# h22hyeon/PC-GNN

Measured on AMD Instinct MI355X. Metric: sampled-nodes/sec, higher is better.
Workload: dtype f32; 1 GPU; yelpchi-like N=45954 F=32 R=3 edges=49315/573616/3402743 endpoints=pareto(2.0) x uniform, PCGNN emb=64 batch=1024 rho=0.5, pick 2*|train_pos|=5346/epoch; global_batch=1024, parallelism=single, engine=graph, epochs_per_launch=4, nodes_processed=1741546

## Files before the change

### pc-gnn_amd/csrc/select.hip

```cpp
#include <limits.h>
#include <stdlib.h>

#include "choose.h"
#include "dense.h"

namespace pcg {

constexpr int KEY_UNROLL = 8;
template <int LEVEL>
__device__ __forceinline__ float s0_ld(const float *__restrict__ s0, uint32_t id) {
    return s0[id];
}
constexpr int KPT = T1_CAP / PCG_WAVE;

#define PCG_STAMP(slot)                                                                \
    do {                                                                               \
        if (a.stamps && tid == 0) a.stamps[(size_t)row * 8 + (slot)] = wall_clock64(); \
    } while (0)

template <int NW>
__device__ __forceinline__ void grp_sync() {
    if constexpr (NW > 1) __syncthreads();
}

template <int NW>
__device__ __forceinline__ void grp_scan(int v, int wave, int lane, int *red, int &prefix, int &total) {
    if constexpr (NW == 1) {
        prefix = 0;
        total = v;
    } else {
        if (lane == 0) red[wave] = v;
        __syncthreads();
        int p = 0, t = 0;
#pragma unroll
        for (int w = 0; w < NW; ++w) {
            const int x = red[w];
            if (w < wave) p += x;
            t += x;
        }
        __syncthreads();
        prefix = p;
        total = t;
    }
}

__device__ __forceinline__ uint32_t wave_min_u32(uint32_t v) {
    uint32_t t;
    t = dpp_u32<0xB1>(v); v = t < v ? t : v;
    t = dpp_u32<0x4E>(v); v = t < v ? t : v;
    t = dpp_u32<0x141>(v); v = t < v ? t : v;
    t = dpp_u32<0x140>(v); v = t < v ? t : v;
    const uint32_t r0 = (uint32_t)__builtin_amdgcn_readlane((int)v, 0), r1 = (uint32_t)__builtin_amdgcn_readlane((int)v, 16);
    const uint32_t r2 = (uint32_t)__builtin_amdgcn_readlane((int)v, 32), r3 = (uint32_t)__builtin_amdgcn_readlane((int)v, 48);
    const uint32_t x = r0 < r1 ? r0 : r1, y = r2 < r3 ? r2 : r3;
    return x < y ? x : y;
}
__device__ __forceinline__ uint32_t wave_max_u32(uint32_t v) {
    uint32_t t;
    t = dpp_u32<0xB1>(v); v = t > v ? t : v;
    t = dpp_u32<0x4E>(v); v = t > v ? t : v;
    t = dpp_u32<0x141>(v); v = t > v ? t : v;
    t = dpp_u32<0x140>(v); v = t > v ? t : v;
    const uint32_t r0 = (uint32_t)__builtin_amdgcn_readlane((int)v, 0), r1 = (uint32_t)__builtin_amdgcn_readlane((int)v, 16);
    const uint32_t r2 = (uint32_t)__builtin_amdgcn_readlane((int)v, 32), r3 = (uint32_t)__builtin_amdgcn_readlane((int)v, 48);
    const uint32_t x = r0 > r1 ? r0 : r1, y = r2 > r3 ? r2 : r3;
    return x > y ? x : y;
}
__device__ __forceinline__ bool sorted_contains(const uint32_t *list, int n, uint32_t x) {
    int lo = 0, hi = n;
    while (lo < hi) {
        const int mid = (lo + hi) >> 1;
        if (list[mid] < x) lo = mid + 1;
        else hi = mid;
    }
    return lo < n && list[lo] == x;
}

constexpr int SORT_SPIN_MAX = 1 << 21;
constexpr int KIDX_MAX = 512;
__device__ __forceinline__ uint64_t pk_ld(const uint64_t *pk, int i);
__device__ __forceinline__ void wait_sorted_keys(const ChooseArgs &a, int &keys_ok, int lane, int *sortw) {
    if (a.n_sort == 0 || keys_ok) return;
    if (__hip_atomic_load(&sortw[0], __ATOMIC_ACQUIRE, __HIP_MEMORY_SCOPE_WORKGROUP) == 0) {
        int elected = 0;
        if (lane == 0) elected = atomicCAS(&sortw[1], 0, 1) == 0;
        elected = __builtin_amdgcn_readfirstlane(elected);
        if (elected) {
            for (int spins = 0;; ++spins) {
                const unsigned seen = (unsigned)__builtin_amdgcn_readfirstlane(
                    (int)__hip_atomic_load(a.sort_done, __ATOMIC_RELAXED, __HIP_MEMORY_SCOPE_AGENT));
                if (seen >= (unsigned)a.n_sort) break;
                if (spins >= SORT_SPIN_MAX) {
                    if (lane == 0 && a.status) atomicOr(a.status, (uint32_t)PCG_ST_SYNC_TIMEOUT);
                    break;
                }
                __builtin_amdgcn_s_sleep(4);
            }
            __builtin_amdgcn_fence(__ATOMIC_ACQUIRE, "workgroup");
            const int P = a.g.n_pos;
            int stride = 16;
            while ((P + stride - 1) / stride > KIDX_MAX) stride <<= 1;
            const int n_idx = (P + stride - 1) / stride;
            for (int t = lane; t < n_idx; t += PCG_WAVE) sortw[4 + t] = (int)(uint32_t)(pk_ld(a.pos_keys, t * stride) >> 32);
            if (lane == 0) {
                sortw[2] = n_idx;
                sortw[3] = stride;
            }
            if (lane == 0) __hip_atomic_store(&sortw[0], 1, __ATOMIC_RELEASE, __HIP_MEMORY_SCOPE_WORKGROUP);
        } else {
            while (__hip_atomic_load(&sortw[0], __ATOMIC_ACQUIRE, __HIP_MEMORY_SCOPE_WORKGROUP) == 0) __builtin_amdgcn_s_sleep(2);
        }
    }
    __builtin_amdgcn_fence(__ATOMIC_ACQUIRE, "workgroup");
    keys_ok = 1;
}

#ifndef PCG_PK_NT
#define PCG_PK_NT 2
#endif
__device__ __forceinline__ uint64_t pk_ld(const uint64_t *pk, int i) {
#if PCG_PK_NT == 2
    const __amdgpu_buffer_rsrc_t rsrc = __builtin_amdgcn_make_buffer_rsrc(const_cast<uint64_t *>(pk), 0, 0x7FFFFFFF, 0x00020000);
    typedef unsigned int u2 __attribute__((ext_vector_type(2)));
    const u2 v = __builtin_amdgcn_raw_buffer_load_b64(rsrc, i * 8, 0, 16);
    return ((uint64_t)v.y << 32) | v.x;
#elif PCG_PK_NT == 1
    return __builtin_nontemporal_load(pk + i);
#else
    return pk[i];
#endif
}

__device__ __forceinline__ float pos_score(const uint64_t *pk, int i) { return from_orderable((uint32_t)(pk_ld(pk, i) >> 32)); }
__device__ __forceinline__ uint32_t pos_dkey(const uint64_t *pk, int i, float c) { return dist_key(c, pos_score(pk, i)); }

template <class Pred>
__device__ __forceinline__ int wave_partition_point(int lo, int hi, int lane, Pred pred) {
    for (;;) {
        const int n = hi - lo;
        if (n <= 0) return lo;
        if (n <= PCG_WAVE) {
            const int idx = lo + lane;
            return lo + wave_count(idx < hi && pred(idx));
        }
        const int step = (n + PCG_WAVE - 1) >> 6;
        int q = lo + (lane + 1) * step - 1;
        if (q > hi - 1) q = hi - 1;
        const int c = wave_count(pred(q));
        if (c == PCG_WAVE) return hi;
        int qc = lo + (c + 1) * step - 1;
        if (qc > hi - 1) qc = hi - 1;
        if (c > 0) {
            int ql = lo + c * step - 1;
            if (ql > hi - 1) ql = hi - 1;
            lo = ql + 1;
        }
        hi = qc;
    }
}

__device__ __forceinline__ int run_end_fwd(const uint64_t *pk, float c, uint32_t kstar, int i0, int end, int lane) {
    for (int i = i0; i < end; i += PCG_WAVE) {
        const int j = i + lane;
        const bool same = j < end && pos_dkey(pk, j, c) == kstar;
        const uint64_t bad = ~__ballot(same);
        if (bad) {
            const int f = i + (__ffsll((unsigned long long)bad) - 1);
            return f < end ? f : end;
        }
    }
    return end;
}
__device__ __forceinline__ int run_begin_bwd(const uint64_t *pk, float c, uint32_t kstar, int i0, int low, int lane) {
    for (int i = i0; i >= low; i -= PCG_WAVE) {
        const int j = i - lane;
        const bool same = j >= low && pos_dkey(pk, j, c) == kstar;
        const uint64_t bad = ~__ballot(same);
        if (bad) {
            const int f = i - (__ffsll((unsigned long long)bad) - 1);
            return (f >= low ? f : low - 1) + 1;
        }
    }
    return low;
}

__device__ __forceinline__ void wave_kth(uint32_t ck, bool have, int n, int want, uint32_t &kstar, int &need, int &n_equal) {
    int lt = 0, eq = 0;
    for (int j = 0; j < n; ++j) {
        const uint32_t o = (uint32_t)__builtin_amdgcn_readlane((int)ck, j);
        lt += o < ck;
        eq += o == ck;
    }
    const int r = want - 1;
    const uint64_t hit = __ballot(have && lt <= r && r < lt + eq);
    const int src = hit ? __ffsll((unsigned long long)hit) - 1 : 0;
    kstar = (uint32_t)__builtin_amdgcn_readlane((int)ck, src);
    n_equal = __builtin_amdgcn_readlane(eq, src);
    need = want - __builtin_amdgcn_readlane(lt, src);
}

struct MinorWindow {
    int L, R, L2, R2, tau, need_t;
};
__device__ __forceinline__ MinorWindow minority_window(const ChooseArgs &a, int m, float c, int lane, const int *sortw) {
    const uint64_t *__restrict__ pk = a.pos_keys;
    const int P = a.g.n_pos;
    int L, R, L2, R2, tau = INT_MAX, need_t = 0;
    if (m >= P) {
        L = L2 = 0;
        R = R2 = P;
    } else {
        int lo_min = 0, lo_max = P - m;
        if (a.n_sort > 0 && sortw) {
            const int n_idx = sortw[2], stride = sortw[3];
            const uint32_t *ix = reinterpret_cast<const uint32_t *>(sortw + 4);
            const int t = wave_partition_point(0, n_idx, lane, [&](int x) { return from_orderable(ix[x]) < c; });
            const int pc_lo = t > 0 ? (t - 1) * stride + 1 : 0, pc_hi = t * stride < P ? t * stride : P;
            lo_min = pc_lo - m > 0 ? pc_lo - m : 0;
            lo_max = pc_hi < P - m ? pc_hi : P - m;
            lo_max = lo_max < lo_min ? lo_min : lo_max;
        }
        const int lo = wave_partition_point(lo_min, lo_max, lane, [&](int x) {
            return (c - pos_score(pk, x)) > (pos_score(pk, x + m) - c);
        });
        const uint32_t NOKEY = 0xFFFFFFFEu;
        const uint32_t ka = pos_dkey(pk, lo, c), kb = pos_dkey(pk, lo + m - 1, c);
        const uint32_t ka1 = m > 1 ? pos_dkey(pk, lo + 1, c) : NOKEY;
        const uint32_t kb1 = m > 1 ? pos_dkey(pk, lo + m - 2, c) : NOKEY;
        const uint32_t kl = lo > 0 ? pos_dkey(pk, lo - 1, c) : NOKEY;
        const uint32_t kr = lo + m < P ? pos_dkey(pk, lo + m, c) : NOKEY;
        const uint32_t ks = ka > kb ? ka : kb;
        const bool tie_l = ka == ks, tie_r = kb == ks;
        const bool none_outside = kl != ks && kr != ks;
        if (none_outside && m == 1) {
            L2 = lo;
            L = R = R2 = lo + 1;
        } else if (none_outside && !(tie_l && tie_r) && (tie_l ? ka1 != ks : kb1 != ks)) {
            L2 = L = tie_l ? lo + 1 : lo;
            R = R2 = tie_l ? lo + m : lo + m - 1;
            if (tie_l) L2 = lo; else R2 = lo + m;
        } else {
            L = run_end_fwd(pk, c, ks, lo, lo + m, lane);
            R = (L == lo + m) ? L : run_begin_bwd(pk, c, ks, lo + m - 1, L, lane);
            L2 = run_begin_bwd(pk, c, ks, lo - 1, 0, lane);
            R2 = run_end_fwd(pk, c, ks, lo + m, P, lane);
        }
        need_t = m - (R - L);
        const int T = (L - L2) + (R2 - R);
        if (T == need_t) {
            L = L2;
            R = R2;
            need_t = 0;
        } else if (T > PCG_WAVE) {
            int plo = 0, phi = P - 1;
            while (plo < phi) {
                const int mid = (plo + phi) >> 1;
                int cn = 0;
                for (int i0 = L2; i0 < L; i0 += PCG_WAVE) {
                    const int i = i0 + lane;
                    cn += wave_count(i < L && (int)(uint32_t)pk_ld(pk, i) <= mid);
                }
                for (int i0 = R; i0 < R2; i0 += PCG_WAVE) {
                    const int i = i0 + lane;
                    cn += wave_count(i < R2 && (int)(uint32_t)pk_ld(pk, i) <= mid);
                }
                if (cn >= need_t) phi = mid;
                else plo = mid + 1;
            }
            tau = plo;
        } else {
            const int nl = L - L2;
            const int ti = lane < nl ? L2 + lane : R + (lane - nl);
            const bool tv = lane < T;
            const int tp = tv ? (int)(uint32_t)pk_ld(pk, ti) : INT_MAX;
            int rank = 0;
            for (int j = 0; j < T; ++j) rank += __builtin_amdgcn_readlane(tp, j) < tp;
            const uint64_t hit = __ballot(tv && rank == need_t - 1);
            const int src = __ffsll((unsigned long long)hit) - 1;
            tau = __builtin_amdgcn_readlane(tp, src < 0 ? 0 : src);
        }
    }
    MinorWindow w;
    w.L = L; w.R = R; w.L2 = L2; w.R2 = R2; w.tau = tau; w.need_t = need_t;
    return w;
}

template <int NW>
__device__ __forceinline__ void finish_row(const ChooseArgs &a, int row, const RowRec &p, float c, const uint32_t *sel, int ns,
                                           bool sel_stored, int wave, int lane, int *red, int &keys_ok, int *sortw,
                                           const int *pre_window = nullptr) {
    constexpr int NT = NW * PCG_WAVE;
    const int tid = wave * PCG_WAVE + lane;
    const int m = p.m, node = p.node;
    int32_t *__restrict__ out = a.w.list + p.lbeg;
    int mt = 0;
    int valid = 0;
    if (m > 0) {
        const uint64_t *__restrict__ pk = a.pos_keys;
        int L, R, L2, R2, tau, need_t;
        if (pre_window) {
            L = pre_window[0]; R = pre_window[1]; L2 = pre_window[2]; R2 = pre_window[3]; tau = pre_window[4]; need_t = pre_window[5];
        } else {
            wait_sorted_keys(a, keys_ok, lane, sortw);
            PCG_STAMP(7);
            const MinorWindow mw = minority_window(a, m, c, lane, sortw);
            L = mw.L; R = mw.R; L2 = mw.L2; R2 = mw.R2; tau = mw.tau; need_t = mw.need_t;
        }
        PCG_STAMP(4);
        const int n_strict = R - L;
        for (int base = tid; base < n_strict; base += NT * KEY_UNROLL) {
            uint32_t pos[KEY_UNROLL], u[KEY_UNROLL];
#pragma unroll
            for (int x = 0; x < KEY_UNROLL; ++x) {
                const int j = base + x * NT;
                pos[x] = (uint32_t)pk_ld(pk, L + (j < n_strict ? j : n_strict - 1));
            }
#pragma unroll
            for (int x = 0; x < KEY_UNROLL; ++x) u[x] = (uint32_t)a.g.train_pos[pos[x]];
#pragma unroll
            for (int x = 0; x < KEY_UNROLL; ++x) {
                const int j = base + x * NT;
                if (j < n_strict) {
                    const bool dup = sorted_contains(sel, ns, u[x]) || (a.add_self && u[x] == (uint32_t)node);
                    out[ns + j] = dup ? -1 : (int32_t)u[x];
                    valid += !dup;
                }
            }
        }
        mt = n_strict;
        if (need_t > 0) {
            int taken = 0;
            for (int part = 0; part < 2; ++part) {
                const int s0i = part == 0 ? L2 : R, e0i = part == 0 ? L : R2;
                for (int i0 = s0i; i0 < e0i; i0 += PCG_WAVE) {
                    const int i = i0 + lane;
                    bool take = false;
                    uint32_t u = 0;
                    if (i < e0i) {
                        const uint32_t pos = (uint32_t)pk_ld(pk, i);
                        take = (int)pos <= tau;
                        if (take) u = (uint32_t)a.g.train_pos[pos];
                    }
                    const uint64_t tmk = __ballot(take);
                    if (take && wave == 0) {
                        const bool dup = sorted_contains(sel, ns, u) || (a.add_self && u == (uint32_t)node);
                        out[ns + n_strict + taken + __popcll(tmk & lanemask_lt())] = dup ? -1 : (int32_t)u;
                        valid += !dup;
                    }
                    taken += __popcll(tmk);
                }
            }
            mt += taken;
        }
    }
    PCG_STAMP(5);
    int n_self = 0;
    if (a.add_self && !sorted_contains(sel, ns, (uint32_t)node)) {
        n_self = 1;
        if (tid == 0) out[ns + mt] = node;
    }
    int vsum = valid;
    for (int o = 1; o < PCG_WAVE; o <<= 1) vsum += __shfl_xor(vsum, o);
    int vpre, vtot;
    grp_scan<NW>(vsum, wave, lane, red, vpre, vtot);
    if (!sel_stored)
        for (int i = tid; i < ns; i += NT) out[i] = (int32_t)sel[i];
    const int used = ns + mt + n_self;
    const int nch = (rec_cap(p, a.add_self) + CHUNK - 1) / CHUNK;
    for (int j = tid; j < nch; j += NT) {
        const int left = used - j * CHUNK;
        a.w.chunk_desc[p.chunk0 + j].z = left < 0 ? 0 : (left > CHUNK ? CHUNK : left);
    }
    if (tid == 0) {
        a.w.len[row] = used;
        a.cnt[row] = ns + vtot + n_self;
    }
    grp_sync<NW>();
    PCG_STAMP(6);
}

__device__ __forceinline__ void report_plain_row(const ChooseArgs &a, int row, const RowRec &p, int ns) {
    a.w.len[row] = ns;
    a.cnt[row] = ns;
    const int nch = (rec_cap(p, 0) + CHUNK - 1) / CHUNK;
    for (int j = 0; j < nch; ++j) {
        const int left = ns - j * CHUNK;
        a.w.chunk_desc[p.chunk0 + j].z = left < 0 ? 0 : (left > CHUNK ? CHUNK : left);
    }
}

#define PCG_ROR_STEP(N)                                                                                     \
    do {                                                                                                    \
        const uint32_t ok = (uint32_t)__builtin_amdgcn_update_dpp(0, (int)key, 0x120 + (N), 0xF, 0xF, false); \
        const int op = __builtin_amdgcn_update_dpp(0, pos, 0x120 + (N), 0xF, 0xF, false);                  \
        rank += (ok < key) || (ok == key && op < pos);                                                      \
    } while (0)

__device__ __forceinline__ void select_four_short_rows(const ChooseArgs &a, int q_first, int na, const int32_t *const *t_indices,
                                                       int lane) {
    const int g = lane >> 4, pos = lane & 15;
    const int qi = q_first + g;
    const bool active = qi < na;
    const int row = a.w.qa[active ? qi : na - 1];
    const RowRec p = a.w.recs[row];
    const int r = row / a.B;
    const int32_t *__restrict__ nbr = t_indices[r] + (p.d > 0 ? p.start : 0);
    const bool have = active && pos < p.d;
    const uint32_t id = (uint32_t)nbr[pos < p.d ? pos : (p.d > 0 ? p.d - 1 : 0)];
    const float c = a.center_s0 ? a.center_s0[row - r * a.B] : a.s0[p.node + a.center_off];
    const bool keep_all = rec_keep_all(p);
    const float sc = s0_ld<2>(a.s0, id);
    const uint32_t key = have ? dist_key(c, sc) : 0xFFFFFFFFu;
    int rank = 0;
    PCG_ROR_STEP(1); PCG_ROR_STEP(2); PCG_ROR_STEP(3); PCG_ROR_STEP(4); PCG_ROR_STEP(5);
    PCG_ROR_STEP(6); PCG_ROR_STEP(7); PCG_ROR_STEP(8); PCG_ROR_STEP(9); PCG_ROR_STEP(10);
    PCG_ROR_STEP(11); PCG_ROR_STEP(12); PCG_ROR_STEP(13); PCG_ROR_STEP(14); PCG_ROR_STEP(15);
    const bool sel = have && (keep_all || rank < p.k);
    const uint32_t gm = (uint32_t)(__ballot(sel) >> (16 * g)) & 0xFFFFu;
    if (sel) a.w.list[p.lbeg + __popc(gm & ((1u << pos) - 1u))] = (int32_t)id;
    if (active && pos == 0) report_plain_row(a, row, p, __popc(gm));
}

__device__ __forceinline__ void select_lane_row(const ChooseArgs &a, int row, uint32_t *area, int lane, int &keys_ok, int *sortw) {
    const int tid = lane;
    if (a.stamps && tid == 0) a.stamps[(size_t)row * 8] = wall_clock64() | ((unsigned long long)blockIdx.x << 54);
    const RowRec p = a.w.recs[row];
    const int d = p.d, k = p.k;
    const bool keep_all = rec_keep_all(p);
    const int r = row / a.B;
    const int32_t *__restrict__ nbr = a.g.indices[r] + (d > 0 ? p.start : 0);
    const float c = a.center_s0 ? a.center_s0[row - r * a.B] : a.s0[p.node + a.center_off];
    uint32_t *sel_lds = area + HIST_W;
    const bool tail = p.m > 0 || a.add_self;
    const bool have = lane < d;
    const uint32_t id = (uint32_t)nbr[have ? lane : (d > 0 ? d - 1 : 0)];
    const float sc = s0_ld<2>(a.s0, id);
    const uint32_t mine = have ? dist_key(c, sc) : 0xFFFFFFFFu;
    PCG_STAMP(1);
    int rank = 0;
    if (!keep_all) {
        for (int j = 0; j < d; ++j)
            rank += (uint32_t)__builtin_amdgcn_readlane((int)mine, j) < mine;
        int sum = have ? rank : 0;
        sum += (int)dpp_u32<0xB1>((uint32_t)sum);
        sum += (int)dpp_u32<0x4E>((uint32_t)sum);
        sum += (int)dpp_u32<0x141>((uint32_t)sum);
        sum += (int)dpp_u32<0x140>((uint32_t)sum);
        const int total = __builtin_amdgcn_readlane(sum, 0) + __builtin_amdgcn_readlane(sum, 16) +
                          __builtin_amdgcn_readlane(sum, 32) + __builtin_amdgcn_readlane(sum, 48);
        if (total != d * (d - 1) / 2)
            for (int j = 0; j < d; ++j)
                rank += ((uint32_t)__builtin_amdgcn_readlane((int)mine, j) == mine) && j < lane;
    }
    const bool s = have && (keep_all || rank < k);
    const uint64_t sm = __ballot(s);
    const int ns = __popcll(sm);
    PCG_STAMP(2);
    if (s) {
        const int at = __popcll(sm & lanemask_lt());
        if (tail) sel_lds[at] = id;
        else a.w.list[p.lbeg + at] = (int32_t)id;
    }
    PCG_STAMP(3);
    if (tail) finish_row<1>(a, row, p, c, sel_lds, ns, false, 0, lane, nullptr, keys_ok, sortw);
    else {
        if (lane == 0) report_plain_row(a, row, p, ns);
        PCG_STAMP(6);
    }
}

__device__ __forceinline__ void select_wave_row(const ChooseArgs &a, int row, uint32_t *area, int lane, int &keys_ok, int *sortw) {
    const int tid = lane;
    if (a.stamps && tid == 0) a.stamps[(size_t)row * 8] = wall_clock64() | ((unsigned long long)blockIdx.x << 54);
    const RowRec p = a.w.recs[row];
    const int d = p.d, k = p.k;
    const bool keep_all = rec_keep_all(p);
    const int r = row / a.B;
    const int32_t *__restrict__ nbr = a.g.indices[r] + p.start;
    const float c = a.center_s0 ? a.center_s0[row - r * a.B] : a.s0[p.node + a.center_off];
    uint32_t *hist = area, *sel_lds = area + HIST_W, *cand = area + HIST_W + T1_CAP;
    const bool tail = p.m > 0 || a.add_self;
    int32_t *__restrict__ out = a.w.list + p.lbeg;

    uint32_t id[KPT], key[KPT];
    {
        float sc[KPT];
#pragma unroll
        for (int u = 0; u < KPT; ++u) {
            const int i = u * PCG_WAVE + lane;
            id[u] = (uint32_t)nbr[i < d ? i : d - 1];
        }
#pragma unroll
        for (int u = 0; u < KPT; ++u) sc[u] = s0_ld<2>(a.s0, id[u]);
#pragma unroll
        for (int u = 0; u < KPT; ++u) key[u] = (u * PCG_WAVE + lane < d) ? dist_key(c, sc[u]) : 0xFFFFFFFFu;
    }
    PCG_STAMP(1);

    uint32_t kstar = 0xFFFFFFFEu;
    int need = 0, n_equal = 0;
    if (!keep_all) {
        uint32_t kmin = 0xFFFFFFFFu, kmax = 0u;
#pragma unroll
        for (int u = 0; u < KPT; ++u)
            if (u * PCG_WAVE + lane < d) {
                kmin = key[u] < kmin ? key[u] : kmin;
                kmax = key[u] > kmax ? key[u] : kmax;
            }
        uint32_t lo = wave_min_u32(kmin), hi = wave_max_u32(kmax);
        int below = 0, cnt = d;
        while (lo < hi && cnt > PCG_WAVE) {
            const uint32_t range = hi - lo;
            const int bits = 32 - __clz((int)range);
            const int shift = bits > 8 ? bits - 8 : 0;
            *reinterpret_cast<uint4 *>(hist + 4 * lane) = make_uint4(0u, 0u, 0u, 0u);
#pragma unroll
            for (int u = 0; u < KPT; ++u)
                if (key[u] >= lo && key[u] <= hi) atomicAdd(&hist[(key[u] - lo) >> shift], 1u);
            const uint4 v = *reinterpret_cast<const uint4 *>(hist + 4 * lane);
            const int s = (int)(v.x + v.y + v.z + v.w);
            const int incl = wave_incl_scan(s, lane);
            const int want = k - below;
            const uint64_t reach = __ballot(incl >= want);
            const int L = __ffsll((unsigned long long)reach) - 1;
            int c0 = incl - s, b = 0, hb = (int)v.x;
            if (c0 + (int)v.x < want) {
                c0 += (int)v.x; b = 1; hb = (int)v.y;
                if (c0 + (int)v.y < want) {
                    c0 += (int)v.y; b = 2; hb = (int)v.z;
                    if (c0 + (int)v.z < want) { c0 += (int)v.z; b = 3; hb = (int)v.w; }
                }
            }
            const int bin = __builtin_amdgcn_readlane(4 * lane + b, L);
            below += __builtin_amdgcn_readlane(c0, L);
            cnt = __builtin_amdgcn_readlane(hb, L);
            lo += (uint32_t)bin << shift;
            const uint32_t top = lo + ((1u << shift) - 1u);
            hi = top < hi ? top : hi;
        }
        kstar = lo;
        need = k - below;
        n_equal = cnt;
        if (lo < hi) {
            int at = 0;
#pragma unroll
            for (int u = 0; u < KPT; ++u) {
                const bool isc = key[u] >= lo && key[u] <= hi;
                const uint64_t bm = __ballot(isc);
                if (isc) cand[at + __popcll(bm & lanemask_lt())] = key[u];
                at += __popcll(bm);
            }
            const bool hv = lane < cnt;
            const uint32_t ck = hv ? cand[lane] : 0xFFFFFFFFu;
            wave_kth(ck, hv, cnt, k - below, kstar, need, n_equal);
        }
    }
    PCG_STAMP(2);

    const bool ranked = n_equal != need;
    int ns = 0, ties_seen = 0;
#pragma unroll
    for (int u = 0; u < KPT; ++u) {
        if (u * PCG_WAVE >= d) break;
        const bool in = u * PCG_WAVE + lane < d;
        bool s = in && key[u] <= kstar;
        if (ranked) {
            const bool tie = in && key[u] == kstar;
            const uint64_t tm = __ballot(tie);
            s = in && (key[u] < kstar || (tie && ties_seen + __popcll(tm & lanemask_lt()) < need));
            ties_seen += __popcll(tm);
        }
        const uint64_t sm = __ballot(s);
        if (s) {
            const int at = ns + __popcll(sm & lanemask_lt());
            if (tail) sel_lds[at] = id[u];
            else out[at] = (int32_t)id[u];
        }
        ns += __popcll(sm);
    }
    PCG_STAMP(3);
    if (tail) finish_row<1>(a, row, p, c, sel_lds, ns, false, 0, lane, nullptr, keys_ok, sortw);
    else {
        if (lane == 0) report_plain_row(a, row, p, ns);
        PCG_STAMP(6);
    }
}

template <bool LDSK, class F>
__device__ __forceinline__ void for_keys(const uint32_t *keys, const uint32_t *__restrict__ gk, int first, int end, int step, F f) {
    if constexpr (LDSK) {
        for (int i = first; i < end; i += step) f(i, keys[i]);
    } else {
        for (int base = first; base < end; base += step * KEY_UNROLL) {
            uint32_t kv[KEY_UNROLL];
#pragma unroll
            for (int u = 0; u < KEY_UNROLL; ++u) {
                const int i = base + u * step;
                kv[u] = gk[i < end ? i : end - 1];
            }
#pragma unroll
            for (int u = 0; u < KEY_UNROLL; ++u) {
                const int i = base + u * step;
                if (i < end) f(i, kv[u]);
            }
        }
    }
}

template <bool LDSK, int NW = SEL_NW>
__device__ __forceinline__ void select_wg_row(const ChooseArgs &a, int row, uint32_t *keys, uint32_t *hist, uint32_t *cand,
                                              int *red, int tid, int &keys_ok, int *sortw, uint32_t *gk = nullptr,
                                              int key_cap = WG_KEYCAP ) {
    constexpr int NT = NW * PCG_WAVE;
    constexpr int HBITS = NW == 8 ? 11 : 12;
    static_assert(4 * NT == (1 << HBITS), "NW is 8 or 16");
    const int lane = tid & (PCG_WAVE - 1), wave = __builtin_amdgcn_readfirstlane(tid >> 6);
    if (a.stamps && tid == 0) a.stamps[(size_t)row * 8] = wall_clock64() | ((unsigned long long)blockIdx.x << 54);
    const RowRec p = a.w.recs[row];
    const int d = p.d, k = p.k;
    const bool keep_all = rec_keep_all(p);
    const int r = row / a.B;
    const int32_t *__restrict__ nbr = a.g.indices[r] + p.start;
    const float *__restrict__ s0 = a.s0;
    const float c = a.center_s0 ? a.center_s0[row - r * a.B] : s0[p.node + a.center_off];
    int32_t *__restrict__ out = a.w.list + p.lbeg;
    int *res = red + 2 * NW + 2;

    uint32_t kstar = 0xFFFFFFFFu;
    int need = 0, n_equal = 0;
    int *win = sortw ? sortw + 4 : nullptr;
    const bool early = !keep_all && p.m > 0 && a.n_sort == 0 && win != nullptr && NW > 1;
    if (!keep_all) {
        uint32_t kmin = 0xFFFFFFFFu, kmax = 0u;
        constexpr int KU1 = 16;
        const int nt1 = early ? NT - PCG_WAVE : NT;
        if (early && wave == NW - 1) {
            const MinorWindow mw = minority_window(a, p.m, c, lane, nullptr);
            if (lane == 0) {
                win[0] = mw.L; win[1] = mw.R; win[2] = mw.L2; win[3] = mw.R2; win[4] = mw.tau; win[5] = mw.need_t;
            }
        } else
        for (int base = tid; base < d; base += nt1 * KU1) {
            uint32_t id[KU1];
            float sc[KU1];
#pragma unroll
            for (int u = 0; u < KU1; ++u) {
                const int i = base + u * nt1;
                id[u] = (uint32_t)nbr[i < d ? i : d - 1];
            }
#pragma unroll
            for (int u = 0; u < KU1; ++u) sc[u] = s0_ld<1>(s0, id[u]);
#pragma unroll
            for (int u = 0; u < KU1; ++u) {
                const int i = base + u * nt1;
                if (i < d) {
                    const uint32_t key = dist_key(c, sc[u]);
                    if constexpr (LDSK) keys[i] = key;
                    else if (gk) gk[i] = key;
                    kmin = key < kmin ? key : kmin;
                    kmax = key > kmax ? key : kmax;
                }
            }
        }
        kmin = wave_min_u32(kmin);
        kmax = wave_max_u32(kmax);
        if (lane == 0) {
            red[wave] = (int)kmin;
            red[NW + wave] = (int)kmax;
        }
        if constexpr (!LDSK) __builtin_amdgcn_fence(__ATOMIC_RELEASE, "workgroup");
        __syncthreads();
        if constexpr (!LDSK) __builtin_amdgcn_fence(__ATOMIC_ACQUIRE, "workgroup");
        for (int w = 0; w < NW; ++w) {
            const uint32_t x = (uint32_t)red[w], y = (uint32_t)red[NW + w];
            kmin = x < kmin ? x : kmin;
            kmax = y > kmax ? y : kmax;
        }
        PCG_STAMP(1);
        uint32_t lo = kmin, hi = kmax;
        int below = 0, cnt = d;
        while (lo < hi && cnt > PCG_WAVE) {
            const uint32_t range = hi - lo;
            const int bits = 32 - __clz((int)range);
            const int shift = bits > HBITS ? bits - HBITS : 0;
            *reinterpret_cast<uint4 *>(hist + 4 * tid) = make_uint4(0u, 0u, 0u, 0u);
            __syncthreads();
            for_keys<LDSK>(keys, gk, tid, d, NT, [&](int, uint32_t key) {
                if (key >= lo && key <= hi) atomicAdd(&hist[(key - lo) >> shift], 1u);
            });
            __syncthreads();
            const uint4 v = *reinterpret_cast<const uint4 *>(hist + 4 * tid);
            const int s = (int)(v.x + v.y + v.z + v.w);
            const int incl_w = wave_incl_scan(s, lane);
            if (lane == PCG_WAVE - 1) red[wave] = incl_w;
            __syncthreads();
            int pre = 0;
#pragma unroll
            for (int w = 0; w < NW; ++w) pre += (w < wave) ? red[w] : 0;
            const int incl = pre + incl_w, excl = incl - s;
            const int want = k - below;
            if (excl < want && want <= incl) {
                int c0 = excl, b = 0, hb = (int)v.x;
                if (c0 + (int)v.x < want) {
                    c0 += (int)v.x; b = 1; hb = (int)v.y;
                    if (c0 + (int)v.y < want) {
                        c0 += (int)v.y; b = 2; hb = (int)v.z;
                        if (c0 + (int)v.z < want) { c0 += (int)v.z; b = 3; hb = (int)v.w; }
                    }
                }
                res[0] = 4 * tid + b;
                res[1] = c0;
                res[2] = hb;
            }
            __syncthreads();
            below += res[1];
            cnt = res[2];
            lo += (uint32_t)res[0] << shift;
            const uint32_t top = lo + ((1u << shift) - 1u);
            hi = top < hi ? top : hi;
        }
        kstar = lo;
        need = k - below;
        n_equal = cnt;
        if (lo < hi) {
            __syncthreads();
            if (tid == 0) res[3] = 0;
            __syncthreads();
            for_keys<LDSK>(keys, gk, tid, d, NT, [&](int, uint32_t key) {
                if (key >= lo && key <= hi) {
                    const int at = atomicAdd(&res[3], 1);
                    if (at < PCG_WAVE) cand[at] = key;
                }
            });
            __syncthreads();
            const bool hv = lane < cnt;
            const uint32_t ck = hv ? cand[lane] : 0xFFFFFFFFu;
            wave_kth(ck, hv, cnt, k - below, kstar, need, n_equal);
        }
        __syncthreads();
    }
    PCG_STAMP(2);

    const bool ranked = !keep_all && n_equal != need;
    const int seg = (((d + NW - 1) / NW) + PCG_WAVE - 1) & ~(PCG_WAVE - 1);
    const int b0 = wave * seg < d ? wave * seg : d;
    const int e0 = b0 + seg < d ? b0 + seg : d;
    int tie_base = 0;
    if (ranked) {
        int tc = 0;
        for_keys<LDSK>(keys, gk, b0 + lane, e0, PCG_WAVE, [&](int, uint32_t key) { tc += key == kstar; });
        for (int o = 1; o < PCG_WAVE; o <<= 1) tc += __shfl_xor(tc, o);
        int ttot;
        grp_scan<NW>(tc, wave, lane, red, tie_base, ttot);
    }
    int ns = 0;
    const bool plain = p.m == 0 && !a.add_self;
    const bool sel_in_lds = (LDSK || (keep_all ? d : k) <= key_cap) && !plain;
    uint32_t *selbuf = sel_in_lds ? keys : reinterpret_cast<uint32_t *>(out);
    if constexpr (LDSK) {
        uint32_t mask = 0;
        int mine = 0, ties_seen = tie_base;
        int it = 0;
        for (int i0 = b0; i0 < e0; i0 += PCG_WAVE, ++it) {
            const int i = i0 + lane;
            const bool in = i < e0;
            const uint32_t key = (in && !keep_all) ? keys[i] : 0u;
            bool s = in && (keep_all || key <= kstar);
            if (ranked) {
                const bool tie = in && key == kstar;
                const uint64_t tm = __ballot(tie);
                s = in && (key < kstar || (tie && ties_seen + __popcll(tm & lanemask_lt()) < need));
                ties_seen += __popcll(tm);
            }
            mask |= (uint32_t)s << it;
            mine += wave_count(s);
        }
        int run;
        grp_scan<NW>(mine, wave, lane, red, run, ns);
        constexpr int CU = 4;
        it = 0;
        for (int i0 = b0; i0 < e0; i0 += CU * PCG_WAVE, it += CU) {
            uint32_t idv[CU];
#pragma unroll
            for (int u = 0; u < CU; ++u) {
                const int i = i0 + u * PCG_WAVE + lane;
                idv[u] = (uint32_t)nbr[i < e0 ? i : d - 1];
            }
#pragma unroll
            for (int u = 0; u < CU; ++u) {
                const bool s = (mask >> (it + u)) & 1u;
                const uint64_t sm = __ballot(s);
                const int at = run + __popcll(sm & lanemask_lt());
                if (s) {
                    if (plain) out[at] = (int32_t)idv[u];
                    else keys[at] = idv[u];
                }
                run += __popcll(sm);
            }
        }
        __syncthreads();
    } else {
        auto stretch_keys = [&](int i0, uint32_t (&id)[KEY_UNROLL], uint32_t (&key)[KEY_UNROLL]) __attribute__((always_inline)) {
#pragma unroll
            for (int u = 0; u < KEY_UNROLL; ++u) {
                const int i = i0 + u * PCG_WAVE + lane;
                id[u] = (uint32_t)nbr[i < e0 ? i : d - 1];
                key[u] = gk[i < e0 ? i : d - 1];
            }
        };
        int mine = 0, ties_seen = tie_base;
        for (int i0 = b0; i0 < e0; i0 += PCG_WAVE * KEY_UNROLL) {
            uint32_t id[KEY_UNROLL], key[KEY_UNROLL];
            stretch_keys(i0, id, key);
#pragma unroll
            for (int u = 0; u < KEY_UNROLL; ++u) {
                const int i = i0 + u * PCG_WAVE + lane;
                const bool in = i < e0;
                bool s = in && (keep_all || key[u] <= kstar);
                if (ranked) {
                    const bool tie = in && key[u] == kstar;
                    const uint64_t tm = __ballot(tie);
                    s = in && (key[u] < kstar || (tie && ties_seen + __popcll(tm & lanemask_lt()) < need));
                    ties_seen += __popcll(tm);
                }
                mine += wave_count(s);
            }
        }
        int run;
        grp_scan<NW>(mine, wave, lane, red, run, ns);
        ties_seen = tie_base;
        for (int i0 = b0; i0 < e0; i0 += PCG_WAVE * KEY_UNROLL) {
            uint32_t id[KEY_UNROLL], key[KEY_UNROLL];
            stretch_keys(i0, id, key);
#pragma unroll
            for (int u = 0; u < KEY_UNROLL; ++u) {
                const int i = i0 + u * PCG_WAVE + lane;
                const bool in = i < e0;
                bool s = in && (keep_all || key[u] <= kstar);
                if (ranked) {
                    const bool tie = in && key[u] == kstar;
                    const uint64_t tm = __ballot(tie);
                    s = in && (key[u] < kstar || (tie && ties_seen + __popcll(tm & lanemask_lt()) < need));
                    ties_seen += __popcll(tm);
                }
                const uint64_t sm = __ballot(s);
                if (s) selbuf[run + __popcll(sm & lanemask_lt())] = id[u];
                run += __popcll(sm);
            }
        }
        __builtin_amdgcn_fence(__ATOMIC_RELEASE, "workgroup");
        __syncthreads();
        __builtin_amdgcn_fence(__ATOMIC_ACQUIRE, "workgroup");
    }
    PCG_STAMP(3);
    if (plain) {
        if (wave == 0) {
            if (lane == 0) {
                a.w.len[row] = ns;
                a.cnt[row] = ns;
            }
            const int nch = (rec_cap(p, 0) + CHUNK - 1) / CHUNK;
            for (int j = lane; j < nch; j += PCG_WAVE) {
                const int left = ns - j * CHUNK;
                a.w.chunk_desc[p.chunk0 + j].z = left < 0 ? 0 : (left > CHUNK ? CHUNK : left);
            }
        }
        PCG_STAMP(6);
        return;
    }
    if constexpr (LDSK) finish_row<NW>(a, row, p, c, keys, ns, false, wave, lane, red, keys_ok, sortw, early ? win : nullptr);
    else finish_row<NW>(a, row, p, c, selbuf, ns, !sel_in_lds, wave, lane, red, keys_ok, sortw, early ? win : nullptr);
}

#ifndef PCG_WG_ROW_PRIO
#define PCG_WG_ROW_PRIO 2
#endif
constexpr int SEL_SHARDS = 8;
constexpr int SORT_TILE = 4096;

template <int TILE, int NW = SEL_NW>
__device__ __forceinline__ void sort_share(const ChooseArgs &a, int w, uint64_t *sh, int *part, int tid) {
    static_assert(TILE % (NW * PCG_WAVE) == 0, "every thread loads the same number of keys of a tile");
    constexpr int PER = TILE / (NW * PCG_WAVE);
    const int lane = tid & (PCG_WAVE - 1), wave = tid >> 6;
    const int P = a.g.n_pos;
    const int group = w % a.n_sort, slice = w / a.n_sort;
    const int i = group * PCG_WAVE + lane;
    const uint64_t *__restrict__ raw = a.raw_keys;
    const uint64_t mine = raw[i < P ? i : P - 1] | (i < P ? 0ull : ~0ull);
    const int jb = slice * a.sort_slice_len;
    const int je = jb + a.sort_slice_len < P ? jb + a.sort_slice_len : P;
    int c = 0;
    for (int t0 = jb; t0 < je; t0 += TILE) {
        const int nt = je - t0 < TILE ? je - t0 : TILE;
        uint64_t kt[PER];
#pragma unroll
        for (int u = 0; u < PER; ++u) {
            const int t = tid + u * NW * PCG_WAVE;
            kt[u] = raw[t0 + (t < nt ? t : nt - 1)] | (t < nt ? 0ull : ~0ull);
        }
        __syncthreads();
#pragma unroll
        for (int u = 0; u < PER; ++u) sh[tid + u * NW * PCG_WAVE] = kt[u];
        __syncthreads();
        const int chunk = (((nt + NW - 1) / NW) + 7) & ~7;
        const int j0 = wave * chunk;
        const int nt8 = (nt + 7) & ~7;
        const int j1 = j0 + chunk < nt8 ? j0 + chunk : nt8;
        const uint4 *sh4 = reinterpret_cast<const uint4 *>(sh);
        for (int j = j0; j < j1; j += 8) {
            const uint4 q0 = sh4[(j >> 1) + 0], q1 = sh4[(j >> 1) + 1], q2 = sh4[(j >> 1) + 2], q3 = sh4[(j >> 1) + 3];
            const uint64_t a0 = ((uint64_t)q0.y << 32) | q0.x, a1 = ((uint64_t)q0.w << 32) | q0.z;
            const uint64_t a2 = ((uint64_t)q1.y << 32) | q1.x, a3 = ((uint64_t)q1.w << 32) | q1.z;
            const uint64_t a4 = ((uint64_t)q2.y << 32) | q2.x, a5 = ((uint64_t)q2.w << 32) | q2.z;
            const uint64_t a6 = ((uint64_t)q3.y << 32) | q3.x, a7 = ((uint64_t)q3.w << 32) | q3.z;
            c += (a0 < mine) + (a1 < mine) + (a2 < mine) + (a3 < mine) + (a4 < mine) + (a5 < mine) + (a6 < mine) + (a7 < mine);
        }
    }
    part[wave * PCG_WAVE + lane] = c;
    __syncthreads();
    if (wave == 0) {
        int cnt = 0;
#pragma unroll
        for (int x = 0; x < NW; ++x) cnt += part[x * PCG_WAVE + lane];
        uint32_t ticket = 0;
        if (a.sort_slices > 1) {
            if (i < P) __hip_atomic_fetch_add(a.rank_acc + i, (uint32_t)cnt, __ATOMIC_RELAXED, __HIP_MEMORY_SCOPE_AGENT);
            asm volatile("s_waitcnt vmcnt(0)" ::: "memory");
            if (lane == 0) ticket = __hip_atomic_fetch_add(a.group_ticket + group, 1u, __ATOMIC_RELAXED, __HIP_MEMORY_SCOPE_AGENT);
            ticket = (uint32_t)__builtin_amdgcn_readfirstlane((int)ticket);
        }
        if (ticket == (uint32_t)a.sort_slices - 1u) {
            if (i < P) {
                uint32_t rank = (uint32_t)cnt;
                if (a.sort_slices > 1) {
                    rank = __hip_atomic_load(a.rank_acc + i, __ATOMIC_RELAXED, __HIP_MEMORY_SCOPE_AGENT);
                    __hip_atomic_store(a.rank_acc + i, 0u, __ATOMIC_RELAXED, __HIP_MEMORY_SCOPE_AGENT);
                }
                __hip_atomic_store(reinterpret_cast<unsigned long long *>(a.sort_out) + (rank < (uint32_t)P ? rank : 0u),
                                   (unsigned long long)mine, __ATOMIC_RELAXED, __HIP_MEMORY_SCOPE_AGENT);
            }
            if (group == 0)
                for (int t = P + lane; t < a.sort_cap; t += PCG_WAVE)
                    __hip_atomic_store(reinterpret_cast<unsigned long long *>(a.sort_out) + t, ~0ull, __ATOMIC_RELAXED, __HIP_MEMORY_SCOPE_AGENT);
            if (lane == 0 && a.sort_slices > 1) __hip_atomic_store(a.group_ticket + group, 0u, __ATOMIC_RELAXED, __HIP_MEMORY_SCOPE_AGENT);
            asm volatile("s_waitcnt vmcnt(0)" ::: "memory");
            if (lane == 0) __hip_atomic_fetch_add(a.sort_done, 1u, __ATOMIC_RELAXED, __HIP_MEMORY_SCOPE_AGENT);
            if (a.stamps && lane == 0) atomicMax(&a.stamps[(size_t)a.g.n_rel * a.B * 8 + 5], (unsigned long long)wall_clock64());
        }
    }
    __syncthreads();
}

template <int K, int U>
__device__ __forceinline__ void clf_step_body(const ClfStep c, const float *__restrict__ X, int F, int stride,
                                           const int32_t *__restrict__ nodes, const int32_t *__restrict__ labels, int B,
                                           uint32_t *lds_u, int tid, unsigned long long *st, int cw) {
    typedef float f4 __attribute__((ext_vector_type(4)));
    constexpr int NT = SEL_NW * PCG_WAVE;
    const int NC = 2 * F + 2, NC4 = (NC + 3) & ~3;
    const int lane = tid & (PCG_WAVE - 1), wave = tid >> 6;
    const int lpr = lanes_per_row(stride), rpw = PCG_WAVE / lpr, slot = lane / lpr, sub = lane % lpr, nch = stride >> 2;
    const int n_part = SEL_NW * rpw;
    float *wl = reinterpret_cast<float *>(lds_u);
    float *red = wl + NC4;
    int *idl = reinterpret_cast<int *>(red + n_part * NC4);
    int RB = ((WG_KEYCAP - (n_part + 1) * NC4) / 2) & ~(PCG_WAVE - 1);
    RB = RB < 2 * NT ? RB : 2 * NT;
    int *yl = idl + RB;
    const bool mine = tid < NC;
    const int ic = mine ? tid : 0;
    const float p_old = c.clf_next[ic], m_old = c.m[ic], v_old = c.v[ic];
    const float t = (float)(c.step_counter[0] + (c.t_ahead > 0 ? c.t_ahead : (c.count_step ? 2 : 1)));
    constexpr int NPRE = 2;
    int nb = B < RB ? B : RB;
    int id_pre[NPRE], y_pre[NPRE];
#pragma unroll
    for (int q = 0; q < NPRE; ++q) {
        const int i = tid + q * NT;
        id_pre[q] = nodes[i < nb ? i : nb - 1];
        y_pre[q] = labels[i < nb ? i : nb - 1];
    }
    for (int i = tid; i < NC; i += NT) {
        const float w = i == tid ? p_old : c.clf_next[i];
        wl[i] = w;
        if (cw == 0) c.theta_clf[i] = w;
        if (cw == 0 && c.clf_out) c.clf_out[i] = w;
    }
#pragma unroll
    for (int q = 0; q < NPRE; ++q) {
        const int i = tid + q * NT;
        if (i < nb) {
            idl[i] = id_pre[q];
            yl[i] = y_pre[q];
        }
    }
    __syncthreads();
    if (st && tid == 0) st[0] = wall_clock64();
    bool has[K];
    int chc[K];
    float w0[K][4], w1[K][4];
#pragma unroll
    for (int k = 0; k < K; ++k) {
        const int ch = sub + k * lpr;
        has[k] = ch < nch;
        chc[k] = has[k] ? ch : nch - 1;
#pragma unroll
        for (int j = 0; j < 4; ++j) {
            const int f = 4 * chc[k] + j;
            const bool ok = has[k] && f < F;
            w0[k][j] = ok ? wl[f] : 0.f;
            w1[k][j] = ok ? wl[F + f] : 0.f;
        }
    }
    const float b0 = wl[2 * F], b1 = wl[2 * F + 1];
    float g0[K][4], g1[K][4], gb0 = 0.f, gb1 = 0.f;
#pragma unroll
    for (int k = 0; k < K; ++k)
#pragma unroll
        for (int j = 0; j < 4; ++j) g0[k][j] = g1[k][j] = 0.f;
    const int per_iter = SEL_NW * rpw;
    for (int blk = 0; blk < B; blk += RB) {
        if (blk > 0) {
            nb = B - blk < RB ? B - blk : RB;
            __syncthreads();
            for (int i = tid; i < nb; i += NT) {
                idl[i] = nodes[blk + i];
                yl[i] = labels[blk + i];
            }
            __syncthreads();
        }
        for (int base = wave * rpw; base < nb; base += per_iter * U) {
            f4 x[U][K];
            int y[U];
#pragma unroll
            for (int u = 0; u < U; ++u) {
                const int b = base + u * per_iter + slot;
                const int bc = b < nb ? b : nb - 1;
                y[u] = b < nb ? yl[bc] : -1;
                const float *xrow = X + (size_t)idl[bc] * stride;
#pragma unroll
                for (int k = 0; k < K; ++k) x[u][k] = *reinterpret_cast<const f4 *>(xrow + 4 * chc[k]);
            }
#pragma unroll
            for (int u = 0; u < U; ++u) {
                float p0 = 0.f, p1 = 0.f;
#pragma unroll
                for (int k = 0; k < K; ++k) {
                    p0 = fmaf(x[u][k].x, w0[k][0], p0); p0 = fmaf(x[u][k].y, w0[k][1], p0);
                    p0 = fmaf(x[u][k].z, w0[k][2], p0); p0 = fmaf(x[u][k].w, w0[k][3], p0);
                    p1 = fmaf(x[u][k].x, w1[k][0], p1); p1 = fmaf(x[u][k].y, w1[k][1], p1);
                    p1 = fmaf(x[u][k].z, w1[k][2], p1); p1 = fmaf(x[u][k].w, w1[k][3], p1);
                }
                p0 = score_reduce(p0, lpr);
                p1 = score_reduce(p1, lpr);
                float loss, d0, d1;
                xent2(p0 + b0, p1 + b1, y[u], loss, d0, d1);
                d0 = y[u] >= 0 ? d0 * c.scale : 0.f;
                d1 = y[u] >= 0 ? d1 * c.scale : 0.f;
#pragma unroll
                for (int k = 0; k < K; ++k) {
                    g0[k][0] = fmaf(d0, x[u][k].x, g0[k][0]); g0[k][1] = fmaf(d0, x[u][k].y, g0[k][1]);
                    g0[k][2] = fmaf(d0, x[u][k].z, g0[k][2]); g0[k][3] = fmaf(d0, x[u][k].w, g0[k][3]);
                    g1[k][0] = fmaf(d1, x[u][k].x, g1[k][0]); g1[k][1] = fmaf(d1, x[u][k].y, g1[k][1]);
                    g1[k][2] = fmaf(d1, x[u][k].z, g1[k][2]); g1[k][3] = fmaf(d1, x[u][k].w, g1[k][3]);
                }
                gb0 += d0;
                gb1 += d1;
            }
        }
    }
    if (st && tid == 0) st[1] = wall_clock64();
    {
        float *mine_red = red + (wave * rpw + slot) * NC4;
#pragma unroll
        for (int k = 0; k < K; ++k)
#pragma unroll
            for (int j = 0; j < 4; ++j) {
                const int f = 4 * chc[k] + j;
                if (has[k] && f < F) {
                    mine_red[f] = g0[k][j];
                    mine_red[F + f] = g1[k][j];
                }
            }
        if (sub == 0) {
            mine_red[2 * F] = gb0;
            mine_red[2 * F + 1] = gb1;
        }
    }
    __syncthreads();
    if (st && tid == 0) st[2] = wall_clock64();
    if (c.n_wg > 1) {
        float *slot_out = c.part + (size_t)cw * c.part_stride;
        for (int i = tid; i < NC; i += NT) {
            float g = red[i];
            for (int w = 1; w < n_part; ++w) g += red[w * NC4 + i];
            __hip_atomic_store(slot_out + i, g, __ATOMIC_RELAXED, __HIP_MEMORY_SCOPE_AGENT);
        }
        asm volatile("s_waitcnt vmcnt(0)" ::: "memory");
        __syncthreads();
        int *flag = reinterpret_cast<int *>(red);
        if (tid == 0) flag[0] = __hip_atomic_fetch_add(c.ticket, 1u, __ATOMIC_RELAXED, __HIP_MEMORY_SCOPE_AGENT) == (unsigned)c.n_wg - 1u;
        __syncthreads();
        const bool last = flag[0] != 0;
        __syncthreads();
        if (!last) return;
        for (int i = tid; i < NC; i += NT) {
            float x[8];
#pragma unroll
            for (int w = 0; w < 8; ++w)
                x[w] = __hip_atomic_load(c.part + (size_t)(w < c.n_wg ? w : c.n_wg - 1) * c.part_stride + i, __ATOMIC_RELAXED, __HIP_MEMORY_SCOPE_AGENT);
            float g = x[0];
#pragma unroll
            for (int w = 1; w < 8; ++w) g = w < c.n_wg ? g + x[w] : g;
            red[i] = g;
        }
        if (tid == 0) __hip_atomic_store(c.ticket, 0u, __ATOMIC_RELAXED, __HIP_MEMORY_SCOPE_AGENT);
    }
    const float bc1 = 1.f - powf(c.h.beta1, t), bc2 = 1.f - powf(c.h.beta2, t);
    for (int i = tid; i < NC; i += NT) {
        float g = red[i];
        if (c.n_wg == 1)
            for (int w = 1; w < n_part; ++w) g += red[w * NC4 + i];
        const bool first = i == tid;
        const float p = first ? p_old : wl[i];
        const float mo = first ? m_old : c.m[i], vo = first ? v_old : c.v[i];
        g = fmaf(c.h.wd, p, g);
        const float mi = c.h.beta1 * mo + (1.f - c.h.beta1) * g;
        const float vi = c.h.beta2 * vo + (1.f - c.h.beta2) * g * g;
        c.m[i] = mi;
        c.v[i] = vi;
        const float denom = sqrtf(vi) / sqrtf(bc2) + c.h.eps;
        c.clf_next[i] = p - (c.h.lr / bc1) * (mi / denom);
    }
    if (c.count_step && tid == 0) __hip_atomic_fetch_add(c.count_step, 1, __ATOMIC_RELAXED, __HIP_MEMORY_SCOPE_AGENT);
    __syncthreads();
}

template <int CLF, int NW = SEL_NW>
__device__ __forceinline__ void select_rows_body(const ChooseArgs &a, int blk, int nblk, unsigned char *smem) {
    static_assert(NW == SEL_NW || NW == 2 * SEL_NW, "8 or 16 waves");
    uint32_t *lds = reinterpret_cast<uint32_t *>(smem);
    uint32_t *hist = lds + a.key_cap;
    uint32_t *cand = hist + 4 * NW * PCG_WAVE;
    int *red = reinterpret_cast<int *>(cand + PCG_WAVE);
    int *claim = red + 2 * NW + 6;
    const int32_t **t_indices = reinterpret_cast<const int32_t **>(red + 2 * NW + 8);
    int *sortw = reinterpret_cast<int *>(t_indices + PCG_MAX_REL);
    if (threadIdx.x < PCG_MAX_REL) t_indices[threadIdx.x] = a.g.indices[threadIdx.x < (unsigned)a.g.n_rel ? threadIdx.x : 0];
    const bool leader = threadIdx.x == 0;
    if (leader) sortw[0] = sortw[1] = 0;
    const int n16 = (int)a.w.counters[C_N16], n4 = (int)a.w.counters[C_N4];
    const int n1 = (int)a.w.counters[C_N1], n0 = (int)a.w.counters[C_N0], na = (int)a.w.counters[C_NA];
    const int n_wg = n16 + n4, n_items = n1 + n0 + (na + 3) / 4;
    const int clf_wg = (CLF && a.clf.clf_next) ? a.clf.n_wg : 0;
    const int grid = nblk - clf_wg, bid = blk - clf_wg;
    const int avail = grid - n_wg > grid / 4 ? grid - n_wg : grid / 4;
    int bs = (n_items + avail - 1) / avail;
    bs = bs < 1 ? 1 : (bs > NW ? NW : bs);
    const int n_units = n_wg + (n_items + bs - 1) / bs;
    const bool pull = n_units > grid;
    const int shard = (bid < 0 ? 0 : bid) % SEL_SHARDS;
    uint32_t *head = a.w.heads + 16 * shard;
    if (a.pending_clear && bid == 0 && leader) a.pending_clear[0] = 0u;
    __syncthreads();
    if (CLF && bid < 0) {
        __builtin_amdgcn_s_setprio(3);
        if (a.stamps && leader) a.stamps[(size_t)a.g.n_rel * a.B * 8 + 2] = wall_clock64();
        const int cw = blk;
        const int32_t *cn = a.clf.nodes ? a.clf.nodes : a.nodes, *cl = a.clf.nodes ? a.clf.labels : a.labels;
        const int cB = a.clf.nodes ? a.clf.B : a.B;
        const int per = ((cB + a.clf.n_wg - 1) / a.clf.n_wg + PCG_WAVE - 1) & ~(PCG_WAVE - 1);
        const int r0 = cw * per < cB ? cw * per : cB, r1 = r0 + per < cB ? r0 + per : cB;
        unsigned long long *cst = (a.stamps && cw == 0) ? a.stamps + (size_t)a.g.n_rel * a.B * 8 + 8 : nullptr;
        if ((int)threadIdx.x >= SEL_NW * PCG_WAVE) return;
        if constexpr (CLF == 2) clf_step_body<2, 2>(a.clf, a.g.X, a.g.feat_dim, a.g.feat_stride, cn + r0, cl + r0, r1 - r0, lds, (int)threadIdx.x, cst, cw);
        else if constexpr (CLF == 1) clf_step_body<1, 3>(a.clf, a.g.X, a.g.feat_dim, a.g.feat_stride, cn + r0, cl + r0, r1 - r0, lds, (int)threadIdx.x, cst, cw);
        if (a.stamps && leader) a.stamps[(size_t)a.g.n_rel * a.B * 8 + 3] = wall_clock64();
        return;
    }

    int u = bid;
    if (CLF && NW == SEL_NW && a.n_wg_units > 0) {
        if (u < a.n_wg_units) {
            float(*wred)[256] = reinterpret_cast<float(*)[256]>(lds + ((int)threadIdx.x >> 8) * 1024);
            const int n_tiles = wgrad_tiles(a.wg.F, a.wg.E, a.wg.R, 0);
            const int tile = 2 * u + ((int)threadIdx.x >> 8);
            wgrad_adam_body<4>(a.wg, tile < n_tiles ? tile : n_tiles - 1, wred, (int)threadIdx.x & 255);
            __syncthreads();
        }
        u = u < a.n_wg_units ? grid - a.n_wg_units + u : u - a.n_wg_units;
    }
    if (a.n_sort > 0) {
        const int helpers = a.n_sort * a.sort_slices;
        if (u < helpers) {
            if (a.stamps && leader && u == 0) a.stamps[(size_t)a.g.n_rel * a.B * 8 + 4] = wall_clock64();
            __builtin_amdgcn_s_setprio(3);
            if (a.sort_slice_len <= 512 * NW / SEL_NW) sort_share<512 * NW / SEL_NW, NW>(a, u, reinterpret_cast<uint64_t *>(lds), reinterpret_cast<int *>(hist), (int)threadIdx.x);
            else sort_share<SORT_TILE, NW>(a, u, reinterpret_cast<uint64_t *>(lds), reinterpret_cast<int *>(hist), (int)threadIdx.x);
            __builtin_amdgcn_s_setprio(0);
        }
        u = u < helpers ? grid - helpers + u : u - helpers;
    }
    int keys_ok = 0;
    int pending = 0, slot = 0;
    while (u < n_units) {
        const bool ahead = u >= n_wg;
        if (leader && pull && ahead) pending = grid + shard + SEL_SHARDS * (int)atomicAdd(head, 1u);
        int tid = (int)threadIdx.x;
        asm volatile("" : "+v"(tid));
        const int lane = tid & (PCG_WAVE - 1), wave = __builtin_amdgcn_readfirstlane(tid >> 6);
        uint32_t *area = lds + wave * WAVE_AREA;
        if (u < n_wg) {
            const int row = __builtin_amdgcn_readfirstlane(u < n16 ? a.w.q16[u] : a.w.q4[u - n16]);
            const int d = a.w.recs[row].d;
            static_assert(true, "");
            if (PCG_WG_ROW_PRIO) __builtin_amdgcn_s_setprio(PCG_WG_ROW_PRIO);
            if (d <= a.key_cap) select_wg_row<true, NW>(a, row, lds, hist, cand, red, tid, keys_ok, sortw, nullptr, a.key_cap);
            if (PCG_WG_ROW_PRIO) __builtin_amdgcn_s_setprio(0);
        } else {
            const int j = wave < bs ? (u - n_wg) * bs + wave : n_items;
            if (j < n1) {
                select_wave_row(a, __builtin_amdgcn_readfirstlane(a.w.q1[j]), area, lane, keys_ok, sortw);
            } else if (j < n1 + n0) {
                select_lane_row(a, __builtin_amdgcn_readfirstlane(a.w.q0[j - n1]), area, lane, keys_ok, sortw);
            } else if (j < n_items) {
                select_four_short_rows(a, 4 * (j - n1 - n0), na, t_indices, lane);
            }
        }
        if (!pull) break;
        if (leader) claim[slot] = ahead ? pending : grid + shard + SEL_SHARDS * (int)atomicAdd(head, 1u);
        __syncthreads();
        u = claim[slot];
        slot ^= 1;
    }
    if (leader && pull) {
        const unsigned done = atomicAdd(a.w.heads + 15, 1u);
        if (done == (unsigned)grid - 1u) {
            for (int i = 0; i < SEL_SHARDS; ++i) atomicExch(a.w.heads + 16 * i, 0u);
            atomicExch(a.w.heads + 15, 0u);
        }
    }
}

template <int CLF>
__global__ void __launch_bounds__(SEL_NW *PCG_WAVE) __attribute__((amdgpu_waves_per_eu(6, 8))) select_rows(const ChooseArgs a) {
    extern __shared__ __align__(16) unsigned char smem[];
    select_rows_body<CLF>(a, (int)blockIdx.x, (int)gridDim.x, smem);
}

template <int CLF>
__global__ void __launch_bounds__(SEL_NW *PCG_WAVE) clf_step_kernel(const ClfStep c, const float *__restrict__ X, int F, int stride) {
    extern __shared__ __align__(16) unsigned char smem[];
    uint32_t *lds = reinterpret_cast<uint32_t *>(smem);
    const int cw = (int)blockIdx.x;
    const int per = ((c.B + c.n_wg - 1) / c.n_wg + PCG_WAVE - 1) & ~(PCG_WAVE - 1);
    const int r0 = cw * per < c.B ? cw * per : c.B, r1 = r0 + per < c.B ? r0 + per : c.B;
    if constexpr (CLF == 2) clf_step_body<2, 2>(c, X, F, stride, c.nodes + r0, c.labels + r0, r1 - r0, lds, (int)threadIdx.x, nullptr, cw);
    else clf_step_body<1, 3>(c, X, F, stride, c.nodes + r0, c.labels + r0, r1 - r0, lds, (int)threadIdx.x, nullptr, cw);
}

int launch_clf_step(const ClfStep &c, const pcg_graph_desc &g, hipStream_t st) {
    if (!c.clf_next || !c.nodes || !c.labels || c.B < 1 || c.n_wg < 1 || c.n_wg > 8 || c.n_wg > (c.B + 1023) / 1024 || g.feat_stride > 512)
        return PCG_E_ARG;
    if (c.n_wg > 1 && (!c.part || !c.ticket)) return PCG_E_ARG;
    const size_t smem = sizeof(uint32_t) * WG_KEYCAP;
    if (g.feat_stride > 256) hipLaunchKernelGGL(clf_step_kernel<2>, dim3(c.n_wg), dim3(SEL_NW * PCG_WAVE), smem, st, c, g.X, g.feat_dim, g.feat_stride);
    else hipLaunchKernelGGL(clf_step_kernel<1>, dim3(c.n_wg), dim3(SEL_NW * PCG_WAVE), smem, st, c, g.X, g.feat_dim, g.feat_stride);
    PCG_LAUNCH_CHECK();
    return PCG_OK;
}

constexpr int LONG_BLOCKS = 256;
__global__ void __launch_bounds__(LONG_NW *PCG_WAVE) select_long_rows(const ChooseArgs a, int64_t per_wg) {
    extern __shared__ __align__(16) unsigned char smem[];
    uint32_t *lds = reinterpret_cast<uint32_t *>(smem);
    uint32_t *hist = lds + LONG_KEYCAP;
    uint32_t *cand = hist + 4 * LONG_NW * PCG_WAVE;
    int *red = reinterpret_cast<int *>(cand + PCG_WAVE);
    const int n16 = (int)a.w.counters[C_N16];
    uint32_t *gk = a.w.key_scratch ? a.w.key_scratch + (size_t)blockIdx.x * per_wg : nullptr;
    int *claim = red + 2 * LONG_NW + 6;
    uint32_t *cursor = a.w.heads + 14, *done = a.w.heads + 13;
    const bool leader = threadIdx.x == 0;
    int u = (int)blockIdx.x, slot = 0;
    int keys_ok = 1;
    while (u < n16) {
        const int row = __builtin_amdgcn_readfirstlane(a.w.q16[u]);
        const int d = a.w.recs[row].d;
        if (d > LONG_KEYCAP) select_wg_row<false, LONG_NW>(a, row, lds, hist, cand, red, (int)threadIdx.x, keys_ok, nullptr, gk, LONG_KEYCAP);
        else if (d > a.key_cap) select_wg_row<true, LONG_NW>(a, row, lds, hist, cand, red, (int)threadIdx.x, keys_ok, nullptr, nullptr, LONG_KEYCAP);
        __syncthreads();
        if (leader) claim[slot] = (int)gridDim.x + (int)atomicAdd(cursor, 1u);
        __syncthreads();
        u = claim[slot];
        slot ^= 1;
    }
    if (leader) {
        const unsigned fin = atomicAdd(done, 1u);
        if (fin == gridDim.x - 1) {
            atomicExch(cursor, 0u);
            atomicExch(done, 0u);
        }
    }
}

static size_t select_smem_bytes(int key_cap, int nw = SEL_NW) {
    return sizeof(uint32_t) * (key_cap + 4 * nw * PCG_WAVE + PCG_WAVE) + sizeof(int) * (2 * nw + 8) + sizeof(void *) * PCG_MAX_REL +
           sizeof(int) * (4 + KIDX_MAX);
}

static int select_sort_shape(ChooseArgs &as, int row_blocks) {
    const ChooseArgs &a = as;
    if (a.n_sort > 0) {
        if (a.n_sort > row_blocks) return PCG_E_ARG;
        static int knob = -1;
        if (knob < 0) {
            const char *e = getenv("PCG_SORT_SLICES");
            knob = e ? atoi(e) : 0;
        }
        int slices = knob > 0 ? knob : 3;
        if (slices > row_blocks / a.n_sort) slices = row_blocks / a.n_sort;
        const int most = (a.g.n_pos + 127) / 128;
        slices = slices > most ? most : slices;
        as.sort_slices = slices < 1 ? 1 : slices;
        as.sort_slice_len = (a.g.n_pos + as.sort_slices - 1) / as.sort_slices;
    }
    return PCG_OK;
}

int launch_select_rows(const ChooseArgs &a, hipStream_t st) {
    static_assert(HIST_WG == 4 * SEL_NW * PCG_WAVE, "one uint4 of bins per thread");
    static_assert(HIST_W == 4 * PCG_WAVE, "one uint4 of bins per lane");
    static_assert(WAVE_AREA >= HIST_W + T1_CAP + PCG_WAVE, "a wave's LDS area: histogram | kept ids | candidates");
    static_assert(((BIG_KEYCAP / SEL_NW + PCG_WAVE - 1) / PCG_WAVE) <= 32, "pass A keeps one bit per iteration in a uint32");
    static_assert((2 * SEL_NW + 8) % 2 == 0, "the pointer table behind red stays 8-byte aligned");
    static_assert(SORT_TILE * 2 <= WG_KEYCAP && SEL_NW * PCG_WAVE <= HIST_WG, "the in-kernel sort's tile and partial counts fit the row paths' LDS");
    static int blocks = 0;
    if (!blocks) {
        const char *e = getenv("PCG_SEL_BLOCKS");
        const int v = e ? atoi(e) : 0;
        blocks = (v >= SEL_SHARDS && v <= SEL_BLOCKS && v % SEL_SHARDS == 0) ? v : SEL_BLOCKS;
    }
    ChooseArgs as = a;
    static int big_knob = -1;
    if (big_knob < 0) {
        const char *e = getenv("PCG_SEL_BIG");
        big_knob = e ? atoi(e) : 0;
    }
    const bool big = big_knob && a.g.max_degree > WG_KEYCAP;
    as.key_cap = big ? BIG_KEYCAP : WG_KEYCAP;
    const int nblk = big ? (blocks > 512 ? 512 : blocks) : blocks;
    const size_t smem = select_smem_bytes(as.key_cap);
    if (big) {
        static bool attr_big = false;
        if (!attr_big) {
            const void *ks[3] = {reinterpret_cast<const void *>(select_rows<0>), reinterpret_cast<const void *>(select_rows<1>),
                                 reinterpret_cast<const void *>(select_rows<2>)};
            for (const void *k : ks)
                if (hipFuncSetAttribute(k, hipFuncAttributeMaxDynamicSharedMemorySize, (int)smem) != hipSuccess) return PCG_E_LAUNCH;
            attr_big = true;
        }
    }
    const int row_blocks = nblk - (a.clf.clf_next ? a.clf.n_wg : 0);
    const int rc = select_sort_shape(as, row_blocks);
    if (rc != PCG_OK) return rc;
    if (a.clf.clf_next && a.g.feat_stride > 256) hipLaunchKernelGGL(select_rows<2>, dim3(nblk), dim3(SEL_NW * PCG_WAVE), smem, st, as);
    else if (a.clf.clf_next) hipLaunchKernelGGL(select_rows<1>, dim3(nblk), dim3(SEL_NW * PCG_WAVE), smem, st, as);
    else hipLaunchKernelGGL(select_rows<0>, dim3(nblk), dim3(SEL_NW * PCG_WAVE), smem, st, as);
    PCG_LAUNCH_CHECK();
    if (a.g.max_degree > as.key_cap) {
        const int64_t per_wg = a.g.max_degree;
        int64_t nb = LONG_BLOCKS;
        if (a.g.max_degree > LONG_KEYCAP) {
            nb = a.w.scratch_cap / per_wg;
            nb = nb < LONG_BLOCKS ? nb : LONG_BLOCKS;
            if (nb < 1) return PCG_E_ARG;
        }
        static_assert(LONG_KEYCAP == LONG_NW * PCG_WAVE * 32, "pass A of an LDS row keeps one bit per iteration in a uint32");
        const size_t long_smem = sizeof(uint32_t) * (LONG_KEYCAP + 4 * LONG_NW * PCG_WAVE + PCG_WAVE) + sizeof(int) * (2 * LONG_NW + 8);
        static bool attr_done = false;
        if (!attr_done) {
            if (hipFuncSetAttribute(reinterpret_cast<const void *>(select_long_rows), hipFuncAttributeMaxDynamicSharedMemorySize,
                                    (int)long_smem) != hipSuccess)
                return PCG_E_LAUNCH;
            attr_done = true;
        }
        ChooseArgs al = as;
        al.n_sort = 0;
        al.pending_clear = nullptr;
        hipLaunchKernelGGL(select_long_rows, dim3((int)nb), dim3(LONG_NW * PCG_WAVE), long_smem, st, al, per_wg);
        PCG_LAUNCH_CHECK();
    }
    return PCG_OK;
}


template <bool WLDS, int F_, int E_, int R_>
__global__ void __launch_bounds__(DENSE_THREADS) dense_select_kernel(const DenseArgs d, const ChooseArgs s, const int n_sel) {
    extern __shared__ __align__(16) unsigned char smem[];
    const int n_dense = d.n_tile_blocks;
    if ((int)blockIdx.x < n_dense) {
        dense_tile_body<WLDS, F_, E_, R_>(d, (int)blockIdx.x, reinterpret_cast<float *>(smem));
        return;
    }
    if ((int)blockIdx.x >= n_dense + n_sel) {
        uint64_t *sh = reinterpret_cast<uint64_t *>(smem);
        int *part = reinterpret_cast<int *>(sh + DENSE_SORT_TILE);
        rank_sort_body<DENSE_SORT_TILE, DENSE_WAVES, false>(nullptr, nullptr, d.sort_n, d.sort_cap, d.sort_out,
                                                            (int)blockIdx.x - n_dense - n_sel, sh, part, d.sort_raw);
        return;
    }
    select_rows_body<1, DENSE_WAVES>(s, (int)blockIdx.x - n_dense, n_sel, smem);
}

int dense_select_blocks(const pcg_graph_desc &g, int emb, int B) {
    static int max_tiles = -1, n_cu = 0;
    if (max_tiles < 0) {
        const char *e = getenv("PCG_PIPE_MAX_TILES");
        max_tiles = e ? atoi(e) : 128;
        int dev = 0;
        if (hipGetDevice(&dev) != hipSuccess || hipDeviceGetAttribute(&n_cu, hipDeviceAttributeMultiprocessorCount, dev) != hipSuccess)
            n_cu = 0;
    }
    if (B < 1 || emb < 16 || emb % 16 != 0 || g.n_rel < 1 || g.n_rel > PCG_MAX_REL) return 0;
    const int n_tiles = (B + TB - 1) / TB;
    if (n_tiles > max_tiles || g.feat_stride > 256 || g.max_degree > WG_KEYCAP) return 0;
    if (dense_smem_bytes(g.feat_dim, emb, g.n_rel, dense_wlds(g.feat_dim, emb, g.n_rel)) > 160 * 1024) return 0;
    int n_sel = n_cu - n_tiles;
    n_sel = (n_sel > SEL_BLOCKS ? SEL_BLOCKS : n_sel) / SEL_SHARDS * SEL_SHARDS;
    const int n_sort = g.n_pos > 0 && g.n_pos <= RANK_MAX ? (g.n_pos + PCG_WAVE - 1) / PCG_WAVE : 0;
    if (n_sel < 64 || n_sel - 8 < n_sort) return 0;
    return n_sel;
}

int launch_dense_select(const DenseArgs &d, const ChooseArgs &a, int n_sel, hipStream_t st) {
    if (a.g.feat_stride > 256 || a.g.max_degree > WG_KEYCAP || d.n_split != 1 || n_sel < 1) return PCG_E_ARG;
    if (d.sort_raw && (!d.sort_out || d.sort_n < 1 || d.sort_n > RANK_MAX || d.sort_cap < d.sort_n)) return PCG_E_ARG;
    const int n_riders = d.sort_raw ? (d.sort_n + PCG_WAVE - 1) / PCG_WAVE : 0;
    const int clf_wg = a.clf.clf_next ? a.clf.n_wg : 0;
    if (clf_wg && a.clf.nodes && (!a.clf.labels || a.clf.B < 1 || clf_wg > (a.clf.B + 1023) / 1024)) return PCG_E_ARG;
    if (n_sel - clf_wg < 8) return PCG_E_ARG;
    ChooseArgs as = a;
    as.key_cap = DENSE_WAVES * WAVE_AREA;
    const int rc = select_sort_shape(as, n_sel - clf_wg);
    if (rc != PCG_OK) return rc;
    const int F = d.feat_dim, E = d.emb, R = d.n_rel;
    const bool wlds = dense_wlds(F, E, R);
    const size_t dsm = dense_smem_bytes(F, E, R, wlds), ssm = select_smem_bytes(DENSE_WAVES * WAVE_AREA, DENSE_WAVES);
    typedef void (*kern_t)(const DenseArgs, const ChooseArgs, const int);
    kern_t kern;
    if (R == 3 && F == 32 && E == 64 && wlds) kern = dense_select_kernel<true, 32, 64, 3>;
    else if (R == 3 && F == 25 && E == 64 && wlds) kern = dense_select_kernel<true, 25, 64, 3>;
    else if (R == 3 && F == 32 && E == 128 && !wlds) kern = dense_select_kernel<false, 32, 128, 3>;
    else if (R == 3 && F == 25 && E == 128 && !wlds) kern = dense_select_kernel<false, 25, 128, 3>;
    else kern = wlds ? dense_select_kernel<true, 0, 0, 0> : dense_select_kernel<false, 0, 0, 0>;
    static kern_t attr_done[6] = {nullptr, nullptr, nullptr, nullptr, nullptr, nullptr};
    bool seen = false;
    for (kern_t k : attr_done) seen = seen || k == kern;
    if (!seen) {
        if (hipFuncSetAttribute(reinterpret_cast<const void *>(kern), hipFuncAttributeMaxDynamicSharedMemorySize, 160 * 1024) !=
            hipSuccess)
            return PCG_E_LAUNCH;
        for (kern_t &k : attr_done)
            if (!k) {
                k = kern;
                break;
            }
    }
    static_assert(sizeof(uint64_t) * DENSE_SORT_TILE + sizeof(int) * DENSE_THREADS <= 64 * 1024, "the riders' LDS is within every dense shape's");
    hipLaunchKernelGGL(kern, dim3(d.n_tile_blocks + n_sel + n_riders), dim3(DENSE_THREADS), dsm > ssm ? dsm : ssm, st, d, as, n_sel);
    PCG_LAUNCH_CHECK();
    return PCG_OK;
}

}
```

Measured before the change: 24.39 million nodes/s.

## Add pre-sorted key path with eager key index and staged window search

When positive keys are already sorted (n_sort == 0), the select kernels get a PRE template variant. In it, one dedicated wave builds the LDS key index at block start instead of an elected wave spinning for sort completion, and key loads use plain cached loads instead of non-temporal buffer loads. It also adds a staged, software-pipelined window search that issues the next probe loads ahead of the compare. This roughly doubles the kernel instantiations and adds complexity, and the gain depends on how often the pre-sorted path is taken.

```diff
diff --git a/pc-gnn_amd/csrc/select.hip b/pc-gnn_amd/csrc/select.hip
--- a/pc-gnn_amd/csrc/select.hip
+++ b/pc-gnn_amd/csrc/select.hip
@@ -78,8 +78,23 @@
 
 constexpr int SORT_SPIN_MAX = 1 << 21;
 constexpr int KIDX_MAX = 512;
+constexpr int WIN_WORDS = 8;
+template <bool PRE = false>
 __device__ __forceinline__ uint64_t pk_ld(const uint64_t *pk, int i);
+__device__ __forceinline__ int key_index_stride(int P) {
+    int stride = 16;
+    while ((P + stride - 1) / stride > KIDX_MAX) stride <<= 1;
+    return stride;
+}
+template <bool PRE>
 __device__ __forceinline__ void wait_sorted_keys(const ChooseArgs &a, int &keys_ok, int lane, int *sortw) {
+    if constexpr (PRE) {
+        if (keys_ok) return;
+        while (__hip_atomic_load(&sortw[0], __ATOMIC_ACQUIRE, __HIP_MEMORY_SCOPE_WORKGROUP) == 0) __builtin_amdgcn_s_sleep(1);
+        __builtin_amdgcn_fence(__ATOMIC_ACQUIRE, "workgroup");
+        keys_ok = 1;
+        return;
+    }
     if (a.n_sort == 0 || keys_ok) return;
     if (__hip_atomic_load(&sortw[0], __ATOMIC_ACQUIRE, __HIP_MEMORY_SCOPE_WORKGROUP) == 0) {
         int elected = 0;
@@ -98,8 +113,7 @@
             }
             __builtin_amdgcn_fence(__ATOMIC_ACQUIRE, "workgroup");
             const int P = a.g.n_pos;
-            int stride = 16;
-            while ((P + stride - 1) / stride > KIDX_MAX) stride <<= 1;
+            const int stride = key_index_stride(P);
             const int n_idx = (P + stride - 1) / stride;
             for (int t = lane; t < n_idx; t += PCG_WAVE) sortw[4 + t] = (int)(uint32_t)(pk_ld(a.pos_keys, t * stride) >> 32);
             if (lane == 0) {
@@ -118,7 +132,12 @@
 #ifndef PCG_PK_NT
 #define PCG_PK_NT 2
 #endif
+#ifndef PCG_PRE_PLAIN
+#define PCG_PRE_PLAIN 1
+#endif
+template <bool PRE>
 __device__ __forceinline__ uint64_t pk_ld(const uint64_t *pk, int i) {
+    if constexpr (PRE && PCG_PRE_PLAIN) return pk[i];
 #if PCG_PK_NT == 2
     const __amdgpu_buffer_rsrc_t rsrc = __builtin_amdgcn_make_buffer_rsrc(const_cast<uint64_t *>(pk), 0, 0x7FFFFFFF, 0x00020000);
     typedef unsigned int u2 __attribute__((ext_vector_type(2)));
@@ -131,8 +150,21 @@
 #endif
 }
 
-__device__ __forceinline__ float pos_score(const uint64_t *pk, int i) { return from_orderable((uint32_t)(pk_ld(pk, i) >> 32)); }
-__device__ __forceinline__ uint32_t pos_dkey(const uint64_t *pk, int i, float c) { return dist_key(c, pos_score(pk, i)); }
+template <bool PRE>
+__device__ __forceinline__ uint32_t pk_score_bits(const uint64_t *pk, int i) {
+    if constexpr (PRE && PCG_PRE_PLAIN) return reinterpret_cast<const uint32_t *>(pk)[2 * (size_t)i + 1];
+    return (uint32_t)(pk_ld<PRE>(pk, i) >> 32);
+}
+template <bool PRE>
+__device__ __forceinline__ uint32_t pk_score_bits_here(const uint64_t *pk, int i) {
+    if constexpr (PRE && PCG_PRE_PLAIN)
+        return __hip_atomic_load(reinterpret_cast<const uint32_t *>(pk) + 2 * (size_t)i + 1, __ATOMIC_RELAXED, __HIP_MEMORY_SCOPE_WAVEFRONT);
+    return (uint32_t)(pk_ld<PRE>(pk, i) >> 32);
+}
+template <bool PRE = false>
+__device__ __forceinline__ float pos_score(const uint64_t *pk, int i) { return from_orderable(pk_score_bits<PRE>(pk, i)); }
+template <bool PRE = false>
+__device__ __forceinline__ uint32_t pos_dkey(const uint64_t *pk, int i, float c) { return dist_key(c, pos_score<PRE>(pk, i)); }
 
 template <class Pred>
 __device__ __forceinline__ int wave_partition_point(int lo, int hi, int lane, Pred pred) {
@@ -159,10 +191,11 @@
     }
 }
 
+template <bool PRE>
 __device__ __forceinline__ int run_end_fwd(const uint64_t *pk, float c, uint32_t kstar, int i0, int end, int lane) {
     for (int i = i0; i < end; i += PCG_WAVE) {
         const int j = i + lane;
-        const bool same = j < end && pos_dkey(pk, j, c) == kstar;
+        const bool same = j < end && pos_dkey<PRE>(pk, j, c) == kstar;
         const uint64_t bad = ~__ballot(same);
         if (bad) {
             const int f = i + (__ffsll((unsigned long long)bad) - 1);
@@ -171,10 +204,11 @@
     }
     return end;
 }
+template <bool PRE>
 __device__ __forceinline__ int run_begin_bwd(const uint64_t *pk, float c, uint32_t kstar, int i0, int low, int lane) {
     for (int i = i0; i >= low; i -= PCG_WAVE) {
         const int j = i - lane;
-        const bool same = j >= low && pos_dkey(pk, j, c) == kstar;
+        const bool same = j >= low && pos_dkey<PRE>(pk, j, c) == kstar;
         const uint64_t bad = ~__ballot(same);
         if (bad) {
             const int f = i - (__ffsll((unsigned long long)bad) - 1);
@@ -202,33 +236,59 @@
 struct MinorWindow {
     int L, R, L2, R2, tau, need_t;
 };
+constexpr uint32_t WIN_NOKEY = 0xFFFFFFFEu;
+template <bool PRE>
+__device__ __forceinline__ void window_bracket(const ChooseArgs &a, int m, float c, int lane, const int *sortw, int &lo_min, int &lo_max) {
+    const int P = a.g.n_pos;
+    lo_min = 0;
+    lo_max = P - m;
+    if ((PRE || a.n_sort > 0) && sortw) {
+        const int stride = PRE ? key_index_stride(P) : sortw[3], n_idx = PRE ? (P + stride - 1) / stride : sortw[2];
+        const uint32_t *ix = reinterpret_cast<const uint32_t *>(sortw + 4);
+        const int t = wave_partition_point(0, n_idx, lane, [&](int x) { return from_orderable(ix[x]) < c; });
+        const int pc_lo = t > 0 ? (t - 1) * stride + 1 : 0, pc_hi = t * stride < P ? t * stride : P;
+        lo_min = pc_lo - m > 0 ? pc_lo - m : 0;
+        lo_max = pc_hi < P - m ? pc_hi : P - m;
+        lo_max = lo_max < lo_min ? lo_min : lo_max;
+    }
+}
+
+template <bool PRE>
+__device__ __forceinline__ MinorWindow window_resolve(const ChooseArgs &a, int m, float c, int lane, int lo, uint32_t ka, uint32_t kb,
+                                                      uint32_t ka1, uint32_t kb1, uint32_t kl, uint32_t kr);
+
+template <bool PRE>
 __device__ __forceinline__ MinorWindow minority_window(const ChooseArgs &a, int m, float c, int lane, const int *sortw) {
     const uint64_t *__restrict__ pk = a.pos_keys;
     const int P = a.g.n_pos;
+    if (m >= P) {
+        MinorWindow w;
+        w.L = w.L2 = 0;
+        w.R = w.R2 = P;
+        w.tau = INT_MAX;
+        w.need_t = 0;
+        return w;
+    }
+    int lo_min, lo_max;
+    window_bracket<PRE>(a, m, c, lane, sortw, lo_min, lo_max);
+    const int lo = wave_partition_point(lo_min, lo_max, lane, [&](int x) {
+        return (c - pos_score<PRE>(pk, x)) > (pos_score<PRE>(pk, x + m) - c);
+    });
+    const uint32_t ka = pos_dkey<PRE>(pk, lo, c), kb = pos_dkey<PRE>(pk, lo + m - 1, c);
+    const uint32_t ka1 = m > 1 ? pos_dkey<PRE>(pk, lo + 1, c) : WIN_NOKEY;
+    const uint32_t kb1 = m > 1 ? pos_dkey<PRE>(pk, lo + m - 2, c) : WIN_NOKEY;
+    const uint32_t kl = lo > 0 ? pos_dkey<PRE>(pk, lo - 1, c) : WIN_NOKEY;
+    const uint32_t kr = lo + m < P ? pos_dkey<PRE>(pk, lo + m, c) : WIN_NOKEY;
+    return window_resolve<PRE>(a, m, c, lane, lo, ka, kb, ka1, kb1, kl, kr);
+}
+
+template <bool PRE>
+__device__ __forceinline__ MinorWindow window_resolve(const ChooseArgs &a, int m, float c, int lane, int lo, uint32_t ka, uint32_t kb,
+                                                      uint32_t ka1, uint32_t kb1, uint32_t kl, uint32_t kr) {
+    const uint64_t *__restrict__ pk = a.pos_keys;
+    const int P = a.g.n_pos;
     int L, R, L2, R2, tau = INT_MAX, need_t = 0;
-    if (m >= P) {
-        L = L2 = 0;
-        R = R2 = P;
-    } else {
-        int lo_min = 0, lo_max = P - m;
-        if (a.n_sort > 0 && sortw) {
-            const int n_idx = sortw[2], stride = sortw[3];
-            const uint32_t *ix = reinterpret_cast<const uint32_t *>(sortw + 4);
-            const int t = wave_partition_point(0, n_idx, lane, [&](int x) { return from_orderable(ix[x]) < c; });
-            const int pc_lo = t > 0 ? (t - 1) * stride + 1 : 0, pc_hi = t * stride < P ? t * stride : P;
-            lo_min = pc_lo - m > 0 ? pc_lo - m : 0;
-            lo_max = pc_hi < P - m ? pc_hi : P - m;
-            lo_max = lo_max < lo_min ? lo_min : lo_max;
-        }
-        const int lo = wave_partition_point(lo_min, lo_max, lane, [&](int x) {
-            return (c - pos_score(pk, x)) > (pos_score(pk, x + m) - c);
-        });
-        const uint32_t NOKEY = 0xFFFFFFFEu;
-        const uint32_t ka = pos_dkey(pk, lo, c), kb = pos_dkey(pk, lo + m - 1, c);
-        const uint32_t ka1 = m > 1 ? pos_dkey(pk, lo + 1, c) : NOKEY;
-        const uint32_t kb1 = m > 1 ? pos_dkey(pk, lo + m - 2, c) : NOKEY;
-        const uint32_t kl = lo > 0 ? pos_dkey(pk, lo - 1, c) : NOKEY;
-        const uint32_t kr = lo + m < P ? pos_dkey(pk, lo + m, c) : NOKEY;
+    {
         const uint32_t ks = ka > kb ? ka : kb;
         const bool tie_l = ka == ks, tie_r = kb == ks;
         const bool none_outside = kl != ks && kr != ks;
@@ -240,10 +300,10 @@
             R = R2 = tie_l ? lo + m : lo + m - 1;
             if (tie_l) L2 = lo; else R2 = lo + m;
         } else {
-            L = run_end_fwd(pk, c, ks, lo, lo + m, lane);
-            R = (L == lo + m) ? L : run_begin_bwd(pk, c, ks, lo + m - 1, L, lane);
-            L2 = run_begin_bwd(pk, c, ks, lo - 1, 0, lane);
-            R2 = run_end_fwd(pk, c, ks, lo + m, P, lane);
+            L = run_end_fwd<PRE>(pk, c, ks, lo, lo + m, lane);
+            R = (L == lo + m) ? L : run_begin_bwd<PRE>(pk, c, ks, lo + m - 1, L, lane);
+            L2 = run_begin_bwd<PRE>(pk, c, ks, lo - 1, 0, lane);
+            R2 = run_end_fwd<PRE>(pk, c, ks, lo + m, P, lane);
         }
         need_t = m - (R - L);
         const int T = (L - L2) + (R2 - R);
@@ -258,11 +318,11 @@
                 int cn = 0;
                 for (int i0 = L2; i0 < L; i0 += PCG_WAVE) {
                     const int i = i0 + lane;
-                    cn += wave_count(i < L && (int)(uint32_t)pk_ld(pk, i) <= mid);
+                    cn += wave_count(i < L && (int)(uint32_t)pk_ld<PRE>(pk, i) <= mid);
                 }
                 for (int i0 = R; i0 < R2; i0 += PCG_WAVE) {
                     const int i = i0 + lane;
-                    cn += wave_count(i < R2 && (int)(uint32_t)pk_ld(pk, i) <= mid);
+                    cn += wave_count(i < R2 && (int)(uint32_t)pk_ld<PRE>(pk, i) <= mid);
                 }
                 if (cn >= need_t) phi = mid;
                 else plo = mid + 1;
@@ -272,7 +332,7 @@
             const int nl = L - L2;
             const int ti = lane < nl ? L2 + lane : R + (lane - nl);
             const bool tv = lane < T;
-            const int tp = tv ? (int)(uint32_t)pk_ld(pk, ti) : INT_MAX;
+            const int tp = tv ? (int)(uint32_t)pk_ld<PRE>(pk, ti) : INT_MAX;
             int rank = 0;
             for (int j = 0; j < T; ++j) rank += __builtin_amdgcn_readlane(tp, j) < tp;
             const uint64_t hit = __ballot(tv && rank == need_t - 1);
@@ -285,10 +345,102 @@
     return w;
 }
 
-template <int NW>
+__device__ __forceinline__ int pp_probe(int lo, int hi, int lane, bool &valid) {
+    const int n = hi - lo;
+    if (n <= PCG_WAVE) {
+        valid = lo + lane < hi;
+        return valid ? lo + lane : hi - 1;
+    }
+    const int step = (n + PCG_WAVE - 1) >> 6;
+    const int q = lo + (lane + 1) * step - 1;
+    valid = true;
+    return q > hi - 1 ? hi - 1 : q;
+}
+__device__ __forceinline__ bool pp_advance(int &lo, int &hi, int cnt) {
+    const int n = hi - lo;
+    if (n <= PCG_WAVE) {
+        lo += cnt;
+        return true;
+    }
+    if (cnt == PCG_WAVE) {
+        lo = hi;
+        return true;
+    }
+    const int step = (n + PCG_WAVE - 1) >> 6;
+    int qc = lo + (cnt + 1) * step - 1;
+    if (qc > hi - 1) qc = hi - 1;
+    if (cnt > 0) {
+        int ql = lo + cnt * step - 1;
+        if (ql > hi - 1) ql = hi - 1;
+        lo = ql + 1;
+    }
+    hi = qc;
+    return hi <= lo;
+}
+
+struct WinStage {
+    int live, lo, hi;
+    uint32_t v0, v1;
+};
+template <bool PRE>
+__device__ __forceinline__ WinStage win_stage_issue(const ChooseArgs &a, int m, int lane, int lo, int hi) {
+    const uint64_t *__restrict__ pk = a.pos_keys;
+    const int P = a.g.n_pos;
+    const bool probe = hi > lo;
+    bool valid;
+    const int x = pp_probe(lo, probe ? hi : lo + 1, lane, valid);
+    int e = lane == 0 ? lo : lane == 1 ? lo + m - 1 : lane == 2 ? lo + 1 : lane == 3 ? lo + m - 2 : lane == 4 ? lo - 1 : lo + m;
+    e = e < 0 ? 0 : (e > P - 1 ? P - 1 : e);
+    WinStage s;
+    s.lo = lo;
+    s.hi = hi;
+    s.live = probe ? 1 : 2;
+    s.v0 = pk_score_bits_here<PRE>(pk, probe ? x : e);
+    s.v1 = pk_score_bits_here<PRE>(pk, probe ? x + m : e);
+    return s;
+}
+__device__ __forceinline__ bool win_stageable(const ChooseArgs &a, int m) {
+    const int P = a.g.n_pos;
+    return m > 0 && m < P && key_index_stride(P) - 1 + m <= PCG_WAVE * PCG_WAVE;
+}
+template <bool PRE>
+__device__ __forceinline__ WinStage win_stage_begin(const ChooseArgs &a, int m, float c, int lane, const int *sortw) {
+    int lo, hi;
+    window_bracket<PRE>(a, m, c, lane, sortw, lo, hi);
+    lo = __builtin_amdgcn_readfirstlane(lo);
+    hi = __builtin_amdgcn_readfirstlane(hi);
+    return win_stage_issue<PRE>(a, m, lane, lo, hi);
+}
+template <bool PRE>
+__device__ __forceinline__ WinStage win_stage_step(const ChooseArgs &a, int m, float c, int lane, const WinStage &s) {
+    bool valid;
+    (void)pp_probe(s.lo, s.hi > s.lo ? s.hi : s.lo + 1, lane, valid);
+    const bool farther = (c - from_orderable(s.v0)) > (from_orderable(s.v1) - c);
+    const int cnt = wave_count(valid & farther);
+    int lo = s.lo, hi = s.hi > s.lo ? s.hi : s.lo + 1;
+    const bool done = pp_advance(lo, hi, cnt);
+    const bool probed = s.live == 1;
+    lo = probed ? lo : s.lo;
+    hi = probed ? (done ? lo : hi) : s.lo;
+    return win_stage_issue<PRE>(a, m, lane, lo, hi);
+}
+template <bool PRE>
+__device__ __forceinline__ MinorWindow win_stage_end(const ChooseArgs &a, int m, float c, int lane, WinStage s) {
+    while (s.live == 1) s = win_stage_step<PRE>(a, m, c, lane, s);
+    const int P = a.g.n_pos, lo = s.lo;
+    const int dk = (int)dist_key(c, from_orderable(s.v0));
+    const uint32_t ka = (uint32_t)__builtin_amdgcn_readlane(dk, 0), kb = (uint32_t)__builtin_amdgcn_readlane(dk, 1);
+    const uint32_t ka1 = m > 1 ? (uint32_t)__builtin_amdgcn_readlane(dk, 2) : WIN_NOKEY;
+    const uint32_t kb1 = m > 1 ? (uint32_t)__builtin_amdgcn_readlane(dk, 3) : WIN_NOKEY;
+    const uint32_t kl = lo > 0 ? (uint32_t)__builtin_amdgcn_readlane(dk, 4) : WIN_NOKEY;
+    const uint32_t kr = lo + m < P ? (uint32_t)__builtin_amdgcn_readlane(dk, 5) : WIN_NOKEY;
+    return window_resolve<PRE>(a, m, c, lane, lo, ka, kb, ka1, kb1, kl, kr);
+}
+
+template <int NW, bool PRE>
 __device__ __forceinline__ void finish_row(const ChooseArgs &a, int row, const RowRec &p, float c, const uint32_t *sel, int ns,
                                            bool sel_stored, int wave, int lane, int *red, int &keys_ok, int *sortw,
-                                           const int *pre_window = nullptr) {
+                                           bool has_window, const MinorWindow &pre_window) {
     constexpr int NT = NW * PCG_WAVE;
     const int tid = wave * PCG_WAVE + lane;
     const int m = p.m, node = p.node;
@@ -298,12 +450,12 @@
     if (m > 0) {
         const uint64_t *__restrict__ pk = a.pos_keys;
         int L, R, L2, R2, tau, need_t;
-        if (pre_window) {
-            L = pre_window[0]; R = pre_window[1]; L2 = pre_window[2]; R2 = pre_window[3]; tau = pre_window[4]; need_t = pre_window[5];
+        if (has_window) {
+            L = pre_window.L; R = pre_window.R; L2 = pre_window.L2; R2 = pre_window.R2; tau = pre_window.tau; need_t = pre_window.need_t;
         } else {
-            wait_sorted_keys(a, keys_ok, lane, sortw);
+            wait_sorted_keys<PRE>(a, keys_ok, lane, sortw);
             PCG_STAMP(7);
-            const MinorWindow mw = minority_window(a, m, c, lane, sortw);
+            const MinorWindow mw = minority_window<PRE>(a, m, c, lane, sortw);
             L = mw.L; R = mw.R; L2 = mw.L2; R2 = mw.R2; tau = mw.tau; need_t = mw.need_t;
         }
         PCG_STAMP(4);
@@ -313,7 +465,7 @@
 #pragma unroll
             for (int x = 0; x < KEY_UNROLL; ++x) {
                 const int j = base + x * NT;
-                pos[x] = (uint32_t)pk_ld(pk, L + (j < n_strict ? j : n_strict - 1));
+                pos[x] = (uint32_t)pk_ld<PRE>(pk, L + (j < n_strict ? j : n_strict - 1));
             }
 #pragma unroll
             for (int x = 0; x < KEY_UNROLL; ++x) u[x] = (uint32_t)a.g.train_pos[pos[x]];
@@ -337,7 +489,7 @@
                     bool take = false;
                     uint32_t u = 0;
                     if (i < e0i) {
-                        const uint32_t pos = (uint32_t)pk_ld(pk, i);
+                        const uint32_t pos = (uint32_t)pk_ld<PRE>(pk, i);
                         take = (int)pos <= tau;
                         if (take) u = (uint32_t)a.g.train_pos[pos];
                     }
@@ -421,10 +573,11 @@
     if (active && pos == 0) report_plain_row(a, row, p, __popc(gm));
 }
 
-__device__ __forceinline__ void select_lane_row(const ChooseArgs &a, int row, uint32_t *area, int lane, int &keys_ok, int *sortw) {
+template <bool PRE, bool STG>
+__device__ __forceinline__ void select_lane_row_body(const ChooseArgs &a, int row, const RowRec &p, uint32_t *area, int lane, int &keys_ok,
+                                                     int *sortw) {
     const int tid = lane;
     if (a.stamps && tid == 0) a.stamps[(size_t)row * 8] = wall_clock64() | ((unsigned long long)blockIdx.x << 54);
-    const RowRec p = a.w.recs[row];
     const int d = p.d, k = p.k;
     const bool keep_all = rec_keep_all(p);
     const int r = row / a.B;
@@ -434,7 +587,14 @@
     const bool tail = p.m > 0 || a.add_self;
     const bool have = lane < d;
     const uint32_t id = (uint32_t)nbr[have ? lane : (d > 0 ? d - 1 : 0)];
+    WinStage ws = {};
+    const int wm = STG ? __builtin_amdgcn_readfirstlane(p.m) : 0;
+    if constexpr (STG) {
+            wait_sorted_keys<PRE>(a, keys_ok, lane, sortw);
+            ws = win_stage_begin<PRE>(a, wm, c, lane, sortw);
+        }
     const float sc = s0_ld<2>(a.s0, id);
+    if constexpr (STG) ws = win_stage_step<PRE>(a, wm, c, lane, ws);
     const uint32_t mine = have ? dist_key(c, sc) : 0xFFFFFFFFu;
     PCG_STAMP(1);
     int rank = 0;
@@ -462,17 +622,25 @@
         else a.w.list[p.lbeg + at] = (int32_t)id;
     }
     PCG_STAMP(3);
-    if (tail) finish_row<1>(a, row, p, c, sel_lds, ns, false, 0, lane, nullptr, keys_ok, sortw);
-    else {
+    if (tail) {
+        MinorWindow mw = {};
+        constexpr bool staged = STG;
+        if constexpr (STG) {
+            PCG_STAMP(7);
+            mw = win_stage_end<PRE>(a, wm, c, lane, ws);
+        }
+        finish_row<1, PRE>(a, row, p, c, sel_lds, ns, false, 0, lane, nullptr, keys_ok, sortw, staged, mw);
+    } else {
         if (lane == 0) report_plain_row(a, row, p, ns);
         PCG_STAMP(6);
     }
 }
 
-__device__ __forceinline__ void select_wave_row(const ChooseArgs &a, int row, uint32_t *area, int lane, int &keys_ok, int *sortw) {
+template <bool PRE, bool STG>
+__device__ __forceinline__ void select_wave_row_body(const ChooseArgs &a, int row, const RowRec &p, uint32_t *area, int lane, int &keys_ok,
+                                                     int *sortw) {
     const int tid = lane;
     if (a.stamps && tid == 0) a.stamps[(size_t)row * 8] = wall_clock64() | ((unsigned long long)blockIdx.x << 54);
-    const RowRec p = a.w.recs[row];
     const int d = p.d, k = p.k;
     const bool keep_all = rec_keep_all(p);
     const int r = row / a.B;
@@ -483,6 +651,8 @@
     int32_t *__restrict__ out = a.w.list + p.lbeg;
 
     uint32_t id[KPT], key[KPT];
+    WinStage ws = {};
+    const int wm = STG ? __builtin_amdgcn_readfirstlane(p.m) : 0;
     {
         float sc[KPT];
 #pragma unroll
@@ -490,8 +660,13 @@
             const int i = u * PCG_WAVE + lane;
             id[u] = (uint32_t)nbr[i < d ? i : d - 1];
         }
+        if constexpr (STG) {
+            wait_sorted_keys<PRE>(a, keys_ok, lane, sortw);
+            ws = win_stage_begin<PRE>(a, wm, c, lane, sortw);
+        }
 #pragma unroll
         for (int u = 0; u < KPT; ++u) sc[u] = s0_ld<2>(a.s0, id[u]);
+        if constexpr (STG) ws = win_stage_step<PRE>(a, wm, c, lane, ws);
 #pragma unroll
         for (int u = 0; u < KPT; ++u) key[u] = (u * PCG_WAVE + lane < d) ? dist_key(c, sc[u]) : 0xFFFFFFFFu;
     }
@@ -579,11 +754,41 @@
         ns += __popcll(sm);
     }
     PCG_STAMP(3);
-    if (tail) finish_row<1>(a, row, p, c, sel_lds, ns, false, 0, lane, nullptr, keys_ok, sortw);
-    else {
+    if (tail) {
+        MinorWindow mw = {};
+        constexpr bool staged = STG;
+        if constexpr (STG) {
+            PCG_STAMP(7);
+            mw = win_stage_end<PRE>(a, wm, c, lane, ws);
+        }
+        finish_row<1, PRE>(a, row, p, c, sel_lds, ns, false, 0, lane, nullptr, keys_ok, sortw, staged, mw);
+    } else {
         if (lane == 0) report_plain_row(a, row, p, ns);
         PCG_STAMP(6);
     }
+}
+
+template <bool PRE, bool STG>
+__device__ __forceinline__ void select_lane_row(const ChooseArgs &a, int row, uint32_t *area, int lane, int &keys_ok, int *sortw) {
+    const RowRec p = a.w.recs[row];
+    if constexpr (STG) {
+        if (win_stageable(a, __builtin_amdgcn_readfirstlane(p.m))) {
+            select_lane_row_body<PRE, true>(a, row, p, area, lane, keys_ok, sortw);
+            return;
+        }
+    }
+    select_lane_row_body<PRE, false>(a, row, p, area, lane, keys_ok, sortw);
+}
+template <bool PRE, bool STG>
+__device__ __forceinline__ void select_wave_row(const ChooseArgs &a, int row, uint32_t *area, int lane, int &keys_ok, int *sortw) {
+    const RowRec p = a.w.recs[row];
+    if constexpr (STG) {
+        if (win_stageable(a, __builtin_amdgcn_readfirstlane(p.m))) {
+            select_wave_row_body<PRE, true>(a, row, p, area, lane, keys_ok, sortw);
+            return;
+        }
+    }
+    select_wave_row_body<PRE, false>(a, row, p, area, lane, keys_ok, sortw);
 }
 
 template <bool LDSK, class F>
@@ -607,7 +812,7 @@
     }
 }
 
-template <bool LDSK, int NW = SEL_NW>
+template <bool LDSK, int NW = SEL_NW, bool PRE = false>
 __device__ __forceinline__ void select_wg_row(const ChooseArgs &a, int row, uint32_t *keys, uint32_t *hist, uint32_t *cand,
                                               int *red, int tid, int &keys_ok, int *sortw, uint32_t *gk = nullptr,
                                               int key_cap = WG_KEYCAP ) {
@@ -628,14 +833,15 @@
 
     uint32_t kstar = 0xFFFFFFFFu;
     int need = 0, n_equal = 0;
-    int *win = sortw ? sortw + 4 : nullptr;
-    const bool early = !keep_all && p.m > 0 && a.n_sort == 0 && win != nullptr && NW > 1;
+    int *win = sortw ? sortw + 4 + KIDX_MAX : nullptr;
+    const bool early = PRE && !keep_all && p.m > 0 && win != nullptr && NW > 1;
     if (!keep_all) {
         uint32_t kmin = 0xFFFFFFFFu, kmax = 0u;
         constexpr int KU1 = 16;
         const int nt1 = early ? NT - PCG_WAVE : NT;
         if (early && wave == NW - 1) {
-            const MinorWindow mw = minority_window(a, p.m, c, lane, nullptr);
+            wait_sorted_keys<PRE>(a, keys_ok, lane, sortw);
+            const MinorWindow mw = minority_window<PRE>(a, p.m, c, lane, sortw);
             if (lane == 0) {
                 win[0] = mw.L; win[1] = mw.R; win[2] = mw.L2; win[3] = mw.R2; win[4] = mw.tau; win[5] = mw.need_t;
             }
@@ -868,8 +1074,12 @@
         PCG_STAMP(6);
         return;
     }
-    if constexpr (LDSK) finish_row<NW>(a, row, p, c, keys, ns, false, wave, lane, red, keys_ok, sortw, early ? win : nullptr);
-    else finish_row<NW>(a, row, p, c, selbuf, ns, !sel_in_lds, wave, lane, red, keys_ok, sortw, early ? win : nullptr);
+    MinorWindow mw = {};
+    if (early) {
+        mw.L = win[0]; mw.R = win[1]; mw.L2 = win[2]; mw.R2 = win[3]; mw.tau = win[4]; mw.need_t = win[5];
+    }
+    if constexpr (LDSK) finish_row<NW, PRE>(a, row, p, c, keys, ns, false, wave, lane, red, keys_ok, sortw, early, mw);
+    else finish_row<NW, PRE>(a, row, p, c, selbuf, ns, !sel_in_lds, wave, lane, red, keys_ok, sortw, early, mw);
 }
 
 #ifndef PCG_WG_ROW_PRIO
@@ -1137,9 +1347,16 @@
     __syncthreads();
 }
 
-template <int CLF, int NW = SEL_NW>
+#ifndef PCG_STAGE_NW8
+#define PCG_STAGE_NW8 1
+#endif
+#ifndef PCG_STAGE_ROWS
+#define PCG_STAGE_ROWS 1
+#endif
+template <int CLF, int NW = SEL_NW, bool PRE = false>
 __device__ __forceinline__ void select_rows_body(const ChooseArgs &a, int blk, int nblk, unsigned char *smem) {
     static_assert(NW == SEL_NW || NW == 2 * SEL_NW, "8 or 16 waves");
+    constexpr bool STG = PRE && PCG_STAGE_ROWS && (NW > SEL_NW || PCG_STAGE_NW8);
     uint32_t *lds = reinterpret_cast<uint32_t *>(smem);
     uint32_t *hist = lds + a.key_cap;
     uint32_t *cand = hist + 4 * NW * PCG_WAVE;
@@ -1150,6 +1367,8 @@
     if (threadIdx.x < PCG_MAX_REL) t_indices[threadIdx.x] = a.g.indices[threadIdx.x < (unsigned)a.g.n_rel ? threadIdx.x : 0];
     const bool leader = threadIdx.x == 0;
     if (leader) sortw[0] = sortw[1] = 0;
+    const bool idx_wave = PRE && (int)threadIdx.x >= (NW - 1) * PCG_WAVE;
+    const bool idx_keys = PRE && a.train_flag && a.pos_keys && a.g.n_pos > 0;
     const int n16 = (int)a.w.counters[C_N16], n4 = (int)a.w.counters[C_N4];
     const int n1 = (int)a.w.counters[C_N1], n0 = (int)a.w.counters[C_N0], na = (int)a.w.counters[C_NA];
     const int n_wg = n16 + n4, n_items = n1 + n0 + (na + 3) / 4;
@@ -1164,6 +1383,28 @@
     uint32_t *head = a.w.heads + 16 * shard;
     if (a.pending_clear && bid == 0 && leader) a.pending_clear[0] = 0u;
     __syncthreads();
+    if (idx_wave) {
+        if (idx_keys) {
+            const int P = a.g.n_pos, stride = key_index_stride(P), n_idx = (P + stride - 1) / stride;
+            constexpr int KIDX_PER_LANE = KIDX_MAX / PCG_WAVE;
+            uint32_t kix[KIDX_PER_LANE];
+#pragma unroll
+            for (int u = 0; u < KIDX_PER_LANE; ++u) {
+                const int t = u * PCG_WAVE + ((int)threadIdx.x & (PCG_WAVE - 1));
+                kix[u] = pk_score_bits<PRE>(a.pos_keys, t * stride < P ? t * stride : P - 1);
+            }
+#pragma unroll
+            for (int u = 0; u < KIDX_PER_LANE; ++u) {
+                const int t = u * PCG_WAVE + ((int)threadIdx.x & (PCG_WAVE - 1));
+                if (t < n_idx) sortw[4 + t] = (int)kix[u];
+            }
+            if (((int)threadIdx.x & (PCG_WAVE - 1)) == 0) {
+                sortw[2] = n_idx;
+                sortw[3] = stride;
+            }
+        }
+        if (((int)threadIdx.x & (PCG_WAVE - 1)) == 0) __hip_atomic_store(&sortw[0], 1, __ATOMIC_RELEASE, __HIP_MEMORY_SCOPE_WORKGROUP);
+    }
     if (CLF && bid < 0) {
         __builtin_amdgcn_s_setprio(3);
         if (a.stamps && leader) a.stamps[(size_t)a.g.n_rel * a.B * 8 + 2] = wall_clock64();
@@ -1216,14 +1457,14 @@
             const int d = a.w.recs[row].d;
             static_assert(true, "");
             if (PCG_WG_ROW_PRIO) __builtin_amdgcn_s_setprio(PCG_WG_ROW_PRIO);
-            if (d <= a.key_cap) select_wg_row<true, NW>(a, row, lds, hist, cand, red, tid, keys_ok, sortw, nullptr, a.key_cap);
+            if (d <= a.key_cap) select_wg_row<true, NW, PRE>(a, row, lds, hist, cand, red, tid, keys_ok, sortw, nullptr, a.key_cap);
             if (PCG_WG_ROW_PRIO) __builtin_amdgcn_s_setprio(0);
         } else {
             const int j = wave < bs ? (u - n_wg) * bs + wave : n_items;
             if (j < n1) {
-                select_wave_row(a, __builtin_amdgcn_readfirstlane(a.w.q1[j]), area, lane, keys_ok, sortw);
+                select_wave_row<PRE, STG>(a, __builtin_amdgcn_readfirstlane(a.w.q1[j]), area, lane, keys_ok, sortw);
             } else if (j < n1 + n0) {
-                select_lane_row(a, __builtin_amdgcn_readfirstlane(a.w.q0[j - n1]), area, lane, keys_ok, sortw);
+                select_lane_row<PRE, STG>(a, __builtin_amdgcn_readfirstlane(a.w.q0[j - n1]), area, lane, keys_ok, sortw);
             } else if (j < n_items) {
                 select_four_short_rows(a, 4 * (j - n1 - n0), na, t_indices, lane);
             }
@@ -1243,10 +1484,10 @@
     }
 }
 
-template <int CLF>
+template <int CLF, bool PRE>
 __global__ void __launch_bounds__(SEL_NW *PCG_WAVE) __attribute__((amdgpu_waves_per_eu(6, 8))) select_rows(const ChooseArgs a) {
     extern __shared__ __align__(16) unsigned char smem[];
-    select_rows_body<CLF>(a, (int)blockIdx.x, (int)gridDim.x, smem);
+    select_rows_body<CLF, SEL_NW, PRE>(a, (int)blockIdx.x, (int)gridDim.x, smem);
 }
 
 template <int CLF>
@@ -1307,7 +1548,7 @@
 
 static size_t select_smem_bytes(int key_cap, int nw = SEL_NW) {
     return sizeof(uint32_t) * (key_cap + 4 * nw * PCG_WAVE + PCG_WAVE) + sizeof(int) * (2 * nw + 8) + sizeof(void *) * PCG_MAX_REL +
-           sizeof(int) * (4 + KIDX_MAX);
+           sizeof(int) * (4 + KIDX_MAX + WIN_WORDS);
 }
 
 static int select_sort_shape(ChooseArgs &as, int row_blocks) {
@@ -1355,8 +1596,9 @@
     if (big) {
         static bool attr_big = false;
         if (!attr_big) {
-            const void *ks[3] = {reinterpret_cast<const void *>(select_rows<0>), reinterpret_cast<const void *>(select_rows<1>),
-                                 reinterpret_cast<const void *>(select_rows<2>)};
+            const void *ks[6] = {reinterpret_cast<const void *>(select_rows<0, false>), reinterpret_cast<const void *>(select_rows<1, false>),
+                                 reinterpret_cast<const void *>(select_rows<2, false>), reinterpret_cast<const void *>(select_rows<0, true>),
+                                 reinterpret_cast<const void *>(select_rows<1, true>), reinterpret_cast<const void *>(select_rows<2, true>)};
             for (const void *k : ks)
                 if (hipFuncSetAttribute(k, hipFuncAttributeMaxDynamicSharedMemorySize, (int)smem) != hipSuccess) return PCG_E_LAUNCH;
             attr_big = true;
@@ -1365,9 +1607,13 @@
     const int row_blocks = nblk - (a.clf.clf_next ? a.clf.n_wg : 0);
     const int rc = select_sort_shape(as, row_blocks);
     if (rc != PCG_OK) return rc;
-    if (a.clf.clf_next && a.g.feat_stride > 256) hipLaunchKernelGGL(select_rows<2>, dim3(nblk), dim3(SEL_NW * PCG_WAVE), smem, st, as);
-    else if (a.clf.clf_next) hipLaunchKernelGGL(select_rows<1>, dim3(nblk), dim3(SEL_NW * PCG_WAVE), smem, st, as);
-    else hipLaunchKernelGGL(select_rows<0>, dim3(nblk), dim3(SEL_NW * PCG_WAVE), smem, st, as);
+    const bool pre = as.n_sort == 0;
+    const int clf = !a.clf.clf_next ? 0 : a.g.feat_stride > 256 ? 2 : 1;
+    typedef void (*sel_kern_t)(const ChooseArgs);
+    const sel_kern_t kern = clf == 2 ? (pre ? select_rows<2, true> : select_rows<2, false>)
+                          : clf == 1 ? (pre ? select_rows<1, true> : select_rows<1, false>)
+                                     : (pre ? select_rows<0, true> : select_rows<0, false>);
+    hipLaunchKernelGGL(kern, dim3(nblk), dim3(SEL_NW * PCG_WAVE), smem, st, as);
     PCG_LAUNCH_CHECK();
     if (a.g.max_degree > as.key_cap) {
         const int64_t per_wg = a.g.max_degree;
@@ -1396,7 +1642,7 @@
 }
 
 
-template <bool WLDS, int F_, int E_, int R_>
+template <bool WLDS, int F_, int E_, int R_, bool PRE>
 __global__ void __launch_bounds__(DENSE_THREADS) dense_select_kernel(const DenseArgs d, const ChooseArgs s, const int n_sel) {
     extern __shared__ __align__(16) unsigned char smem[];
     const int n_dense = d.n_tile_blocks;
@@ -1411,7 +1657,7 @@
                                                             (int)blockIdx.x - n_dense - n_sel, sh, part, d.sort_raw);
         return;
     }
-    select_rows_body<1, DENSE_WAVES>(s, (int)blockIdx.x - n_dense, n_sel, smem);
+    select_rows_body<1, DENSE_WAVES, PRE>(s, (int)blockIdx.x - n_dense, n_sel, smem);
 }
 
 int dense_select_blocks(const pcg_graph_desc &g, int emb, int B) {
@@ -1450,12 +1696,15 @@
     const size_t dsm = dense_smem_bytes(F, E, R, wlds), ssm = select_smem_bytes(DENSE_WAVES * WAVE_AREA, DENSE_WAVES);
     typedef void (*kern_t)(const DenseArgs, const ChooseArgs, const int);
     kern_t kern;
-    if (R == 3 && F == 32 && E == 64 && wlds) kern = dense_select_kernel<true, 32, 64, 3>;
-    else if (R == 3 && F == 25 && E == 64 && wlds) kern = dense_select_kernel<true, 25, 64, 3>;
-    else if (R == 3 && F == 32 && E == 128 && !wlds) kern = dense_select_kernel<false, 32, 128, 3>;
-    else if (R == 3 && F == 25 && E == 128 && !wlds) kern = dense_select_kernel<false, 25, 128, 3>;
-    else kern = wlds ? dense_select_kernel<true, 0, 0, 0> : dense_select_kernel<false, 0, 0, 0>;
-    static kern_t attr_done[6] = {nullptr, nullptr, nullptr, nullptr, nullptr, nullptr};
+    const bool pre = as.n_sort == 0;
+#define PCG_DS_KERN(W, F, E, R) (pre ? dense_select_kernel<W, F, E, R, true> : dense_select_kernel<W, F, E, R, false>)
+    if (R == 3 && F == 32 && E == 64 && wlds) kern = PCG_DS_KERN(true, 32, 64, 3);
+    else if (R == 3 && F == 25 && E == 64 && wlds) kern = PCG_DS_KERN(true, 25, 64, 3);
+    else if (R == 3 && F == 32 && E == 128 && !wlds) kern = PCG_DS_KERN(false, 32, 128, 3);
+    else if (R == 3 && F == 25 && E == 128 && !wlds) kern = PCG_DS_KERN(false, 25, 128, 3);
+    else kern = wlds ? PCG_DS_KERN(true, 0, 0, 0) : PCG_DS_KERN(false, 0, 0, 0);
+#undef PCG_DS_KERN
+    static kern_t attr_done[12] = {nullptr, nullptr, nullptr, nullptr, nullptr, nullptr, nullptr, nullptr, nullptr, nullptr, nullptr, nullptr};
     bool seen = false;
     for (kern_t k : attr_done) seen = seen || k == kern;
     if (!seen) {
```

Measured after the change: 24.70 million nodes/s (median of 6 runs). +1.2%, better.
